# xmed-lab/GL-Fusion

Hardware: AMD Instinct MI355X
Metric: clips/sec fwd+bwd (B=4, 3 views x16x112x112) per GPU, weak scaling (higher is better)
Workload: dtype f32 (amax-scaled split-fp16 x3 MFMA, fp32 accumulate: fp32-equivalent); 1 GPU; C2: (B,V,T,H,W)=(4,3,16,112,112) per GPU, views 1/3/4, fp32 train() fwd + sum-BCE + bwd; global_batch_clips=4, frames_per_view_per_gpu=64, precision=f16x3, parallelism=single GPU, ranks_in_collective=1

## Files before the change

### gl-fusion_amd/csrc/norm.hip

```cpp
#include "stream_common.h"
#include "split_f16.h"

using namespace glf;

namespace {

constexpr int RT = 256;
constexpr int MAX_SLICES = 1024;

__host__ __device__ inline int n_slices_c(int rows, int c) {
    int s = (rows + 31) / 32;
    int cap = 524288 / (c > 0 ? c : 1);
    if (cap < 128) cap = 128;
    if (cap > MAX_SLICES) cap = MAX_SLICES;
    return s < 1 ? 1 : (s > cap ? cap : s);
}

struct Coef { const float* mean; const float* invstd; const float* gamma; const float* beta; };

struct OpStats {
    const float* x; int ldx;
    __device__ void operator()(int r, int c, float4& a, float4& b) const {
        a = *reinterpret_cast<const float4*>(x + (long long)r * ldx + c);
        b = make_float4(a.x * a.x, a.y * a.y, a.z * a.z, a.w * a.w);
    }
};
struct OpColsum {
    const float* dy; int ld;
    __device__ void operator()(int r, int c, float4& a, float4& b) const {
        a = *reinterpret_cast<const float4*>(dy + (long long)r * ld + c);
        b = make_float4(0.f, 0.f, 0.f, 0.f);
    }
};
__device__ __forceinline__ float bn_val(float x, float mu, float is, float ga, float be) { return (x - mu) * is * ga + be; }

struct OpBnBwd {
    const float* dy; int lddy; const float* x; int ldx; const float* y; int ldy;
    const float* mean; const float* invstd; const float* gamma; const float* beta; int relu;
    const unsigned char* mask; int c4;
    const float* dy2; int lddy2;
    __device__ void operator()(int r, int c, float4& a, float4& b) const {
        a = *reinterpret_cast<const float4*>(dy + (long long)r * lddy + c);
        if (dy2) {
            const float4 a2 = *reinterpret_cast<const float4*>(dy2 + (long long)r * lddy2 + c);
            a.x += a2.x; a.y += a2.y; a.z += a2.z; a.w += a2.w;
        }
        const float4 xx = *reinterpret_cast<const float4*>(x + (long long)r * ldx + c);
        const float4 mu = *reinterpret_cast<const float4*>(mean + c);
        const float4 is = *reinterpret_cast<const float4*>(invstd + c);
        if (relu && mask) {
            const unsigned m = mask[(long long)r * c4 + (c >> 2)];
            a.x = (m & 1u) ? a.x : 0.f; a.y = (m & 2u) ? a.y : 0.f; a.z = (m & 4u) ? a.z : 0.f; a.w = (m & 8u) ? a.w : 0.f;
        } else if (relu) {
            float4 yy;
            if (y) {
                yy = *reinterpret_cast<const float4*>(y + (long long)r * ldy + c);
            } else {
                const float4 ga = *reinterpret_cast<const float4*>(gamma + c);
                const float4 be = *reinterpret_cast<const float4*>(beta + c);
                yy = make_float4(bn_val(xx.x, mu.x, is.x, ga.x, be.x), bn_val(xx.y, mu.y, is.y, ga.y, be.y),
                                 bn_val(xx.z, mu.z, is.z, ga.z, be.z), bn_val(xx.w, mu.w, is.w, ga.w, be.w));
            }
            a.x = yy.x > 0.f ? a.x : 0.f; a.y = yy.y > 0.f ? a.y : 0.f;
            a.z = yy.z > 0.f ? a.z : 0.f; a.w = yy.w > 0.f ? a.w : 0.f;
        }
        b = make_float4(a.x * (xx.x - mu.x) * is.x, a.y * (xx.y - mu.y) * is.y,
                        a.z * (xx.z - mu.z) * is.z, a.w * (xx.w - mu.w) * is.w);
    }
};
struct OpLnParam {
    const float* dz; const float* w; const float* x; Coef bn; const float* row_mean; const float* row_rstd; int c_total;
    __device__ void operator()(int r, int c, float4& a, float4& b) const {
        const long long o = (long long)r * c_total + c;
        b = *reinterpret_cast<const float4*>(dz + o);
        const float4 ww = *reinterpret_cast<const float4*>(w + o);
        const float4 xx = *reinterpret_cast<const float4*>(x + o);
        const float4 mu = *reinterpret_cast<const float4*>(bn.mean + c);
        const float4 is = *reinterpret_cast<const float4*>(bn.invstd + c);
        const float4 ga = *reinterpret_cast<const float4*>(bn.gamma + c);
        const float4 be = *reinterpret_cast<const float4*>(bn.beta + c);
        const float m = row_mean[r], rs = row_rstd[r];
        const float u0 = (ww.x - mu.x) * is.x * ga.x + be.x + xx.x;
        const float u1 = (ww.y - mu.y) * is.y * ga.y + be.y + xx.y;
        const float u2 = (ww.z - mu.z) * is.z * ga.z + be.z + xx.z;
        const float u3 = (ww.w - mu.w) * is.w * ga.w + be.w + xx.w;
        a = make_float4(b.x * (u0 - m) * rs, b.y * (u1 - m) * rs, b.z * (u2 - m) * rs, b.w * (u3 - m) * rs);
    }
};

template <class Op>
__global__ __launch_bounds__(RT) void colreduce_kernel(Op op, int rows, int c, int slices, double* __restrict__ partial) {
    __shared__ double sh_a[RT * 4];
    __shared__ double sh_b[RT * 4];
    const int tid = threadIdx.x;
    const int c4 = c >> 2;
    const int tpr = c4 < RT ? c4 : RT;
    const int rpp = RT / tpr;
    const int ct = tid % tpr, rl = tid / tpr;
    const int slice = blockIdx.x;
    const int per = (rows + slices - 1) / slices;
    const int r0 = slice * per, r1 = min(rows, r0 + per);
    for (int cb = blockIdx.y * tpr; cb < c4; cb += gridDim.y * tpr) {
        const int cc = cb + ct;
        double a0 = 0, a1 = 0, a2 = 0, a3 = 0, b0 = 0, b1 = 0, b2 = 0, b3 = 0;
        if (cc < c4 && rl < rpp) {
            for (int r = r0 + rl; r < r1; r += rpp) {
                float4 a, b;
                op(r, cc * 4, a, b);
                a0 += a.x; a1 += a.y; a2 += a.z; a3 += a.w;
                b0 += b.x; b1 += b.y; b2 += b.z; b3 += b.w;
            }
        }
        sh_a[tid * 4 + 0] = a0; sh_a[tid * 4 + 1] = a1; sh_a[tid * 4 + 2] = a2; sh_a[tid * 4 + 3] = a3;
        sh_b[tid * 4 + 0] = b0; sh_b[tid * 4 + 1] = b1; sh_b[tid * 4 + 2] = b2; sh_b[tid * 4 + 3] = b3;
        __syncthreads();
        if (rl == 0 && cc < c4) {
            for (int q = 1; q < rpp; ++q) {
                const int o = (q * tpr + ct) * 4;
                a0 += sh_a[o]; a1 += sh_a[o + 1]; a2 += sh_a[o + 2]; a3 += sh_a[o + 3];
                b0 += sh_b[o]; b1 += sh_b[o + 1]; b2 += sh_b[o + 2]; b3 += sh_b[o + 3];
            }
            double* pa = partial + (long long)slice * c + cc * 4;
            double* pb = partial + (long long)(slices + slice) * c + cc * 4;
            pa[0] = a0; pa[1] = a1; pa[2] = a2; pa[3] = a3;
            pb[0] = b0; pb[1] = b1; pb[2] = b2; pb[3] = b3;
        }
        __syncthreads();
    }
}

__global__ __launch_bounds__(RT) void bnbwd_reduce_kernel(OpBnBwd op, int rows, int c, int slices, double* __restrict__ partial,
                                                          float* __restrict__ pmax) {
    __shared__ double sh_a[RT * 4];
    __shared__ double sh_b[RT * 4];
    __shared__ float sh_m[RT * 8];
    const int tid = threadIdx.x;
    const int c4 = c >> 2;
    const int tpr = c4 < RT ? c4 : RT;
    const int rpp = RT / tpr;
    const int ct = tid % tpr, rl = tid / tpr;
    const int slice = blockIdx.x;
    const int per = (rows + slices - 1) / slices;
    const int r0 = slice * per, r1 = min(rows, r0 + per);
    for (int cb = blockIdx.y * tpr; cb < c4; cb += gridDim.y * tpr) {
        const int cc = cb + ct;
        double a0 = 0, a1 = 0, a2 = 0, a3 = 0, b0 = 0, b1 = 0, b2 = 0, b3 = 0;
        float mg[4] = {0.f, 0.f, 0.f, 0.f}, mx[4] = {0.f, 0.f, 0.f, 0.f};
        if (cc < c4 && rl < rpp) {
            const float4 mu = *reinterpret_cast<const float4*>(op.mean + cc * 4);
            const float4 is = *reinterpret_cast<const float4*>(op.invstd + cc * 4);
            for (int r = r0 + rl; r < r1; r += rpp) {
                float4 a, b;
                op(r, cc * 4, a, b);
                a0 += a.x; a1 += a.y; a2 += a.z; a3 += a.w;
                b0 += b.x; b1 += b.y; b2 += b.z; b3 += b.w;
                const float4 xx = *reinterpret_cast<const float4*>(op.x + (long long)r * op.ldx + cc * 4);
                mg[0] = fmaxf(mg[0], fabsf(a.x)); mg[1] = fmaxf(mg[1], fabsf(a.y)); mg[2] = fmaxf(mg[2], fabsf(a.z)); mg[3] = fmaxf(mg[3], fabsf(a.w));
                mx[0] = fmaxf(mx[0], fabsf((xx.x - mu.x) * is.x)); mx[1] = fmaxf(mx[1], fabsf((xx.y - mu.y) * is.y));
                mx[2] = fmaxf(mx[2], fabsf((xx.z - mu.z) * is.z)); mx[3] = fmaxf(mx[3], fabsf((xx.w - mu.w) * is.w));
            }
        }
        sh_a[tid * 4 + 0] = a0; sh_a[tid * 4 + 1] = a1; sh_a[tid * 4 + 2] = a2; sh_a[tid * 4 + 3] = a3;
        sh_b[tid * 4 + 0] = b0; sh_b[tid * 4 + 1] = b1; sh_b[tid * 4 + 2] = b2; sh_b[tid * 4 + 3] = b3;
#pragma unroll
        for (int j = 0; j < 4; ++j) { sh_m[tid * 8 + j] = mg[j]; sh_m[tid * 8 + 4 + j] = mx[j]; }
        __syncthreads();
        if (rl == 0 && cc < c4) {
            for (int q = 1; q < rpp; ++q) {
                const int o = (q * tpr + ct) * 4;
                a0 += sh_a[o]; a1 += sh_a[o + 1]; a2 += sh_a[o + 2]; a3 += sh_a[o + 3];
                b0 += sh_b[o]; b1 += sh_b[o + 1]; b2 += sh_b[o + 2]; b3 += sh_b[o + 3];
#pragma unroll
                for (int j = 0; j < 4; ++j) { mg[j] = fmaxf(mg[j], sh_m[2 * o + j]); mx[j] = fmaxf(mx[j], sh_m[2 * o + 4 + j]); }
            }
            double* pa = partial + (long long)slice * c + cc * 4;
            double* pb = partial + (long long)(slices + slice) * c + cc * 4;
            pa[0] = a0; pa[1] = a1; pa[2] = a2; pa[3] = a3;
            pb[0] = b0; pb[1] = b1; pb[2] = b2; pb[3] = b3;
            *reinterpret_cast<float4*>(pmax + (long long)slice * c + cc * 4) = make_float4(mg[0], mg[1], mg[2], mg[3]);
            *reinterpret_cast<float4*>(pmax + (long long)(slices + slice) * c + cc * 4) = make_float4(mx[0], mx[1], mx[2], mx[3]);
        }
        __syncthreads();
    }
}

constexpr int FUSED_TPR = 16;
__host__ __device__ inline int fused_slices(int rows, int c) {
    const int c4 = c > 4 ? c / 4 : 1;
    const int tpr = c4 < FUSED_TPR ? c4 : FUSED_TPR;
    const int rpp = RT / tpr;
    int s = (rows + 16 * rpp - 1) / (16 * rpp);
    const int cblocks = (c4 + tpr - 1) / tpr;
    int cap = 1024 / cblocks;
    if (cap < 1) cap = 1;
    return s < 1 ? 1 : (s > cap ? cap : s);
}
template <bool HAS2, int RM>
__global__ __launch_bounds__(RT) void bnbwd_reduce_atomic_kernel(OpBnBwd op, int rows, int c, int slices, double* __restrict__ sums,
                                                                 float* __restrict__ cmax) {
    __shared__ float sh[RT * 8];
    const int tid = threadIdx.x;
    const int c4 = c >> 2;
    const int tpr = c4 < FUSED_TPR ? c4 : FUSED_TPR;
    const int rpp = RT / tpr;
    const int ct = tid % tpr, rl = tid / tpr;
    const int slice = blockIdx.x;
    const int per = (rows + slices - 1) / slices;
    const int r0 = slice * per, r1 = min(rows, r0 + per);
    for (int cb = blockIdx.y * tpr; cb < c4; cb += gridDim.y * tpr) {
        const int cc = cb + ct;
        float4 sa = make_float4(0.f, 0.f, 0.f, 0.f), sb = sa, mg = sa, mx = sa;
        if (cc < c4 && rl < rpp) {
            const int c0 = cc * 4;
            const float4 mu = *reinterpret_cast<const float4*>(op.mean + c0);
            const float4 is = *reinterpret_cast<const float4*>(op.invstd + c0);
            float4 ga = mu, be = mu;
            if (RM == 2) { ga = *reinterpret_cast<const float4*>(op.gamma + c0); be = *reinterpret_cast<const float4*>(op.beta + c0); }
            auto fold = [&](float4 a, const float4 a2, const float4 xx, const float4 yy, unsigned m) __attribute__((always_inline)) {
                if (HAS2) { a.x += a2.x; a.y += a2.y; a.z += a2.z; a.w += a2.w; }
                if (RM == 2) {
                    m = (bn_val(xx.x, mu.x, is.x, ga.x, be.x) > 0.f ? 1u : 0u) | (bn_val(xx.y, mu.y, is.y, ga.y, be.y) > 0.f ? 2u : 0u) |
                        (bn_val(xx.z, mu.z, is.z, ga.z, be.z) > 0.f ? 4u : 0u) | (bn_val(xx.w, mu.w, is.w, ga.w, be.w) > 0.f ? 8u : 0u);
                } else if (RM == 3) {
                    m = (yy.x > 0.f ? 1u : 0u) | (yy.y > 0.f ? 2u : 0u) | (yy.z > 0.f ? 4u : 0u) | (yy.w > 0.f ? 8u : 0u);
                }
                if (RM != 0) { a.x = (m & 1u) ? a.x : 0.f; a.y = (m & 2u) ? a.y : 0.f; a.z = (m & 4u) ? a.z : 0.f; a.w = (m & 8u) ? a.w : 0.f; }
                const float4 xh = make_float4((xx.x - mu.x) * is.x, (xx.y - mu.y) * is.y, (xx.z - mu.z) * is.z, (xx.w - mu.w) * is.w);
                sa.x += a.x; sa.y += a.y; sa.z += a.z; sa.w += a.w;
                sb.x += a.x * (xx.x - mu.x) * is.x; sb.y += a.y * (xx.y - mu.y) * is.y; sb.z += a.z * (xx.z - mu.z) * is.z; sb.w += a.w * (xx.w - mu.w) * is.w;
                if (cmax) {
                    mg.x = fmaxf(mg.x, fabsf(a.x)); mg.y = fmaxf(mg.y, fabsf(a.y)); mg.z = fmaxf(mg.z, fabsf(a.z)); mg.w = fmaxf(mg.w, fabsf(a.w));
                    mx.x = fmaxf(mx.x, fabsf(xh.x)); mx.y = fmaxf(mx.y, fabsf(xh.y)); mx.z = fmaxf(mx.z, fabsf(xh.z)); mx.w = fmaxf(mx.w, fabsf(xh.w));
                }
            };
            int r = r0 + rl;
            for (; r + 3 * rpp < r1; r += 4 * rpp) {
                float4 qa[4], qa2[4], qx[4], qy[4];
                unsigned m[4] = {15u, 15u, 15u, 15u};
#pragma unroll
                for (int u = 0; u < 4; ++u) {
                    const long long row = r + u * rpp;
                    qa[u] = *reinterpret_cast<const float4*>(op.dy + row * op.lddy + c0);
                    if (HAS2) qa2[u] = *reinterpret_cast<const float4*>(op.dy2 + row * op.lddy2 + c0);
                    qx[u] = *reinterpret_cast<const float4*>(op.x + row * op.ldx + c0);
                    if (RM == 3) qy[u] = *reinterpret_cast<const float4*>(op.y + row * op.ldy + c0);
                    if (RM == 1) m[u] = op.mask[row * op.c4 + cc];
                }
                __builtin_amdgcn_sched_barrier(0);
#pragma unroll
                for (int u = 0; u < 4; ++u) fold(qa[u], HAS2 ? qa2[u] : qa[u], qx[u], RM == 3 ? qy[u] : qx[u], m[u]);
            }
            for (; r < r1; r += rpp) {
                const long long row = r;
                const float4 qa = *reinterpret_cast<const float4*>(op.dy + row * op.lddy + c0);
                const float4 qa2 = HAS2 ? *reinterpret_cast<const float4*>(op.dy2 + row * op.lddy2 + c0) : qa;
                const float4 qx = *reinterpret_cast<const float4*>(op.x + row * op.ldx + c0);
                const float4 qy = RM == 3 ? *reinterpret_cast<const float4*>(op.y + row * op.ldy + c0) : qx;
                const unsigned m = RM == 1 ? op.mask[row * op.c4 + cc] : 15u;
                fold(qa, qa2, qx, qy, m);
            }
        }
        const int ncol = tpr * 4;
        for (int pass = 0; pass < (cmax ? 2 : 1); ++pass) {
            if (rl < rpp) {
                const float4 u = pass == 0 ? sa : mg, v = pass == 0 ? sb : mx;
                float* d0 = sh + (0 * rpp + rl) * ncol + ct * 4;
                float* d1 = sh + (1 * rpp + rl) * ncol + ct * 4;
                d0[0] = u.x; d0[1] = u.y; d0[2] = u.z; d0[3] = u.w;
                d1[0] = v.x; d1[1] = v.y; d1[2] = v.z; d1[3] = v.w;
            }
            __syncthreads();
            for (int idx = tid; idx < 2 * ncol; idx += RT) {
                const int st = idx / ncol, col = idx - st * ncol;
                const int gc = cb * 4 + col;
                if (gc < c) {
                    if (pass == 0) {
                        double d = 0;
                        for (int q = 0; q < rpp; ++q) d += sh[(st * rpp + q) * ncol + col];
                        atomicAdd(sums + st * c + gc, d);
                    } else {
                        float m = 0.f;
                        for (int q = 0; q < rpp; ++q) m = fmaxf(m, sh[(st * rpp + q) * ncol + col]);
                        if (m > 0.f) atomicMax(reinterpret_cast<unsigned*>(cmax + st * c + gc), __float_as_uint(m));
                    }
                }
            }
            __syncthreads();
        }
    }
}

constexpr int FIN_CH = 16, FIN_LANES = 16;

__device__ __forceinline__ void fold_partials(const double* __restrict__ partial, int slices, int c, int ch, int lane,
                                              double& s, double& q, double* sh) {
    s = 0; q = 0;
    if (ch < c) {
        double s1 = 0, q1 = 0, s2 = 0, q2 = 0, s3 = 0, q3 = 0;
        int i = lane;
        for (; i + 3 * FIN_LANES < slices; i += 4 * FIN_LANES) {
            s += partial[(long long)i * c + ch];                     q += partial[(long long)(slices + i) * c + ch];
            s1 += partial[(long long)(i + FIN_LANES) * c + ch];      q1 += partial[(long long)(slices + i + FIN_LANES) * c + ch];
            s2 += partial[(long long)(i + 2 * FIN_LANES) * c + ch];  q2 += partial[(long long)(slices + i + 2 * FIN_LANES) * c + ch];
            s3 += partial[(long long)(i + 3 * FIN_LANES) * c + ch];  q3 += partial[(long long)(slices + i + 3 * FIN_LANES) * c + ch];
        }
        for (; i < slices; i += FIN_LANES) {
            s += partial[(long long)i * c + ch];
            q += partial[(long long)(slices + i) * c + ch];
        }
        s += (s1 + s2) + s3; q += (q1 + q2) + q3;
    }
    const int t = threadIdx.x;
    sh[t] = s; sh[256 + t] = q;
    __syncthreads();
    if (lane == 0) {
        for (int l = 1; l < FIN_LANES; ++l) { s += sh[t + l * FIN_CH]; q += sh[256 + t + l * FIN_CH]; }
    }
}

__global__ __launch_bounds__(256) void bn_stats_finalize(const double* __restrict__ partial, int slices, int c, int rows, float eps,
                                                         float momentum, float* mean, float* invstd, float* rmean, float* rvar, long long* nbt) {
    __shared__ double sh[512];
    const int cx = threadIdx.x % FIN_CH, lane = threadIdx.x / FIN_CH;
    const int ch = blockIdx.x * FIN_CH + cx;
    double s, q;
    fold_partials(partial, slices, c, ch, lane, s, q, sh);
    if (lane != 0 || ch >= c) return;
    if (ch == 0 && nbt) *nbt += 1;
    const double m = s / rows;
    double var = q / rows - m * m;
    if (var < 0) var = 0;
    mean[ch] = (float)m;
    invstd[ch] = (float)(1.0 / sqrt(var + (double)eps));
    if (rmean) {
        const double unb = rows > 1 ? var * rows / (rows - 1) : var;
        rmean[ch] = (1.f - momentum) * rmean[ch] + momentum * (float)m;
        rvar[ch] = (1.f - momentum) * rvar[ch] + momentum * (float)unb;
    }
}

__global__ __launch_bounds__(256) void sum_finalize(const double* __restrict__ partial, int slices, int c, float* out_a, float* out_b) {
    __shared__ double sh[512];
    const int cx = threadIdx.x % FIN_CH, lane = threadIdx.x / FIN_CH;
    const int ch = blockIdx.x * FIN_CH + cx;
    double s, q;
    fold_partials(partial, slices, c, ch, lane, s, q, sh);
    if (lane != 0 || ch >= c) return;
    if (out_a) out_a[ch] = (float)s;
    if (out_b) out_b[ch] = (float)q;
}

__global__ __launch_bounds__(256) void bnbwd_finalize(const double* __restrict__ partial, const float* __restrict__ pmax, int slices, int c,
                                                      const float* __restrict__ gamma, const float* __restrict__ invstd, float inv_n,
                                                      int training, float* out_a, float* out_b, float* __restrict__ bound,
                                                      float* __restrict__ keep) {
    __shared__ double sh[512];
    __shared__ float shm[512];
    const int cx = threadIdx.x % FIN_CH, lane = threadIdx.x / FIN_CH;
    const int ch = blockIdx.x * FIN_CH + cx;
    double s, q;
    fold_partials(partial, slices, c, ch, lane, s, q, sh);
    float mg = 0.f, mx = 0.f;
    if (ch < c) {
        float g1 = 0.f, x1 = 0.f, g2 = 0.f, x2 = 0.f, g3 = 0.f, x3 = 0.f;
        int i = lane;
        for (; i + 3 * FIN_LANES < slices; i += 4 * FIN_LANES) {
            mg = fmaxf(mg, pmax[(long long)i * c + ch]);                      mx = fmaxf(mx, pmax[(long long)(slices + i) * c + ch]);
            g1 = fmaxf(g1, pmax[(long long)(i + FIN_LANES) * c + ch]);        x1 = fmaxf(x1, pmax[(long long)(slices + i + FIN_LANES) * c + ch]);
            g2 = fmaxf(g2, pmax[(long long)(i + 2 * FIN_LANES) * c + ch]);    x2 = fmaxf(x2, pmax[(long long)(slices + i + 2 * FIN_LANES) * c + ch]);
            g3 = fmaxf(g3, pmax[(long long)(i + 3 * FIN_LANES) * c + ch]);    x3 = fmaxf(x3, pmax[(long long)(slices + i + 3 * FIN_LANES) * c + ch]);
        }
        for (; i < slices; i += FIN_LANES) {
            mg = fmaxf(mg, pmax[(long long)i * c + ch]);
            mx = fmaxf(mx, pmax[(long long)(slices + i) * c + ch]);
        }
        mg = fmaxf(fmaxf(mg, g1), fmaxf(g2, g3)); mx = fmaxf(fmaxf(mx, x1), fmaxf(x2, x3));
    }
    shm[threadIdx.x] = mg; shm[256 + threadIdx.x] = mx;
    __syncthreads();
    if (lane != 0 || ch >= c) return;
    for (int l = 1; l < FIN_LANES; ++l) { mg = fmaxf(mg, shm[threadIdx.x + l * FIN_CH]); mx = fmaxf(mx, shm[256 + threadIdx.x + l * FIN_CH]); }
    if (out_a) out_a[ch] = (float)s;
    if (out_b) out_b[ch] = (float)q;
    if (keep) { keep[ch] = (float)s; keep[c + ch] = (float)q; }
    const float k = fabsf(gamma[ch] * invstd[ch]);
    const float b = 1.0001f * k * (training ? mg + inv_n * (fabsf((float)s) + mx * fabsf((float)q)) : mg);
    if (b > 0.f && b < 3.0e38f) atomicMax(reinterpret_cast<unsigned*>(bound), __float_as_uint(b));
}

__global__ void bn_replay_kernel(const float* __restrict__ mean, const float* __restrict__ invstd, int rows, float eps, float momentum,
                                 float* rmean, float* rvar, long long* nbt, int c) {
    const int ch = blockIdx.x * blockDim.x + threadIdx.x;
    if (ch == 0 && nbt) *nbt += 1;
    if (ch >= c) return;
    const double is = (double)invstd[ch];
    double var = 1.0 / (is * is) - (double)eps;
    if (var < 0) var = 0;
    const double unb = rows > 1 ? var * rows / (rows - 1) : var;
    rmean[ch] = (1.f - momentum) * rmean[ch] + momentum * mean[ch];
    rvar[ch] = (1.f - momentum) * rvar[ch] + momentum * (float)unb;
}

__global__ void bn_eval_coeffs_kernel(const float* rm, const float* rv, float eps, float* mean, float* invstd, int c) {
    const int ch = blockIdx.x * blockDim.x + threadIdx.x;
    if (ch >= c) return;
    mean[ch] = rm[ch];
    invstd[ch] = 1.0f / sqrtf(rv[ch] + eps);
}


__global__ __launch_bounds__(256) void bn_apply_kernel(const float* __restrict__ x, int ldx, const float* __restrict__ res, int ldr,
                                                       float* __restrict__ y, int ldy, Coef k, long long total4, int c4, int relu,
                                                       float* __restrict__ amax_out, unsigned char* __restrict__ mask) {
    float am = 0.f;
    for (long long i = blockIdx.x * (long long)blockDim.x + threadIdx.x; i < total4; i += (long long)gridDim.x * blockDim.x) {
        const long long r = i / c4;
        const int c = (int)(i - r * c4) * 4;
        const float4 xx = *reinterpret_cast<const float4*>(x + r * ldx + c);
        const float4 mu = *reinterpret_cast<const float4*>(k.mean + c);
        const float4 is = *reinterpret_cast<const float4*>(k.invstd + c);
        const float4 ga = *reinterpret_cast<const float4*>(k.gamma + c);
        const float4 be = *reinterpret_cast<const float4*>(k.beta + c);
        float4 o = make_float4(bn_val(xx.x, mu.x, is.x, ga.x, be.x), bn_val(xx.y, mu.y, is.y, ga.y, be.y),
                               bn_val(xx.z, mu.z, is.z, ga.z, be.z), bn_val(xx.w, mu.w, is.w, ga.w, be.w));
        if (res) {
            const float4 rr = *reinterpret_cast<const float4*>(res + r * ldr + c);
            o.x += rr.x; o.y += rr.y; o.z += rr.z; o.w += rr.w;
        }
        if (mask) mask[i] = (unsigned char)((o.x > 0.f) | ((o.y > 0.f) << 1) | ((o.z > 0.f) << 2) | ((o.w > 0.f) << 3));
        if (relu) { o.x = fmaxf(o.x, 0.f); o.y = fmaxf(o.y, 0.f); o.z = fmaxf(o.z, 0.f); o.w = fmaxf(o.w, 0.f); }
        *reinterpret_cast<float4*>(y + r * ldy + c) = o;
        am = fmaxf(fmaxf(am, fmaxf(fabsf(o.x), fabsf(o.y))), fmaxf(fabsf(o.z), fabsf(o.w)));
    }
    if (amax_out) block_amax(am, amax_out);
}

constexpr int APPLY_MAX_C = 4096;
__global__ __launch_bounds__(256) void bn_apply_sums_kernel(const float* __restrict__ x, int ldx, const float* __restrict__ res, int ldr,
                                                            float* __restrict__ y, int ldy, const double* __restrict__ sums, int rows, int c,
                                                            float eps, float momentum, const float* __restrict__ gamma, const float* __restrict__ beta,
                                                            float* __restrict__ mean_out, float* __restrict__ invstd_out, float* rmean, float* rvar,
                                                            long long* nbt, long long total4, int c4, int relu, float* __restrict__ amax_out,
                                                            unsigned char* __restrict__ mask, const float* __restrict__ colmax) {
    extern __shared__ __attribute__((aligned(16))) float s_coef[];
    __shared__ float s_bound[4];
    float* s_mean = s_coef;
    float* s_is = s_coef + c;
    float bound = 0.f;
    for (int ch = threadIdx.x; ch < c; ch += blockDim.x) {
        const double m = sums[ch] / rows;
        double var = sums[c + ch] / rows - m * m;
        if (var < 0) var = 0;
        const float mf = (float)m, isf = (float)(1.0 / sqrt(var + (double)eps));
        s_mean[ch] = mf; s_is[ch] = isf;
        if (colmax) bound = fmaxf(bound, fabsf(gamma[ch]) * isf * (colmax[ch] + fabsf(mf)) + fabsf(beta[ch]));
        if (blockIdx.x == 0) {
            mean_out[ch] = mf; invstd_out[ch] = isf;
            if (rmean) {
                const double unb = rows > 1 ? var * rows / (rows - 1) : var;
                rmean[ch] = (1.f - momentum) * rmean[ch] + momentum * (float)m;
                rvar[ch] = (1.f - momentum) * rvar[ch] + momentum * (float)unb;
            }
        }
    }
    if (blockIdx.x == 0 && threadIdx.x == 0 && nbt) *nbt += 1;
    float sc = 1.f, sc_inv = 1.f;
    if (colmax) {
#pragma unroll
        for (int o = 32; o > 0; o >>= 1) bound = fmaxf(bound, __shfl_xor(bound, o, 64));
        if ((threadIdx.x & 63) == 0) s_bound[threadIdx.x >> 6] = bound;
    }
    __syncthreads();
    if (colmax) {
        bound = 1.0001f * fmaxf(fmaxf(s_bound[0], s_bound[1]), fmaxf(s_bound[2], s_bound[3]));
        if (blockIdx.x == 0 && threadIdx.x == 0) *amax_out = bound;
        pow2_scale(&bound, sc, sc_inv);
    }
    float am = 0.f;
    for (long long i = blockIdx.x * (long long)blockDim.x + threadIdx.x; i < total4; i += (long long)gridDim.x * blockDim.x) {
        const long long r = i / c4;
        const int cc = (int)(i - r * c4) * 4;
        const float4 xx = *reinterpret_cast<const float4*>(x + r * ldx + cc);
        const float4 mu = *reinterpret_cast<const float4*>(s_mean + cc);
        const float4 is = *reinterpret_cast<const float4*>(s_is + cc);
        const float4 ga = *reinterpret_cast<const float4*>(gamma + cc);
        const float4 be = *reinterpret_cast<const float4*>(beta + cc);
        float4 o = make_float4(bn_val(xx.x, mu.x, is.x, ga.x, be.x), bn_val(xx.y, mu.y, is.y, ga.y, be.y),
                               bn_val(xx.z, mu.z, is.z, ga.z, be.z), bn_val(xx.w, mu.w, is.w, ga.w, be.w));
        if (res) {
            const float4 rr = *reinterpret_cast<const float4*>(res + r * ldr + cc);
            o.x += rr.x; o.y += rr.y; o.z += rr.z; o.w += rr.w;
        }
        if (mask) mask[i] = (unsigned char)((o.x > 0.f) | ((o.y > 0.f) << 1) | ((o.z > 0.f) << 2) | ((o.w > 0.f) << 3));
        if (relu) { o.x = fmaxf(o.x, 0.f); o.y = fmaxf(o.y, 0.f); o.z = fmaxf(o.z, 0.f); o.w = fmaxf(o.w, 0.f); }
        if (colmax) {
            const SplitH sp = split4h(o, sc);
            const float2 h = __builtin_bit_cast(float2, sp.h), l = __builtin_bit_cast(float2, sp.l);
            o = make_float4(h.x, h.y, l.x, l.y);
        } else {
            am = fmaxf(fmaxf(am, fmaxf(fabsf(o.x), fabsf(o.y))), fmaxf(fabsf(o.z), fabsf(o.w)));
        }
        *reinterpret_cast<float4*>(y + r * ldy + cc) = o;
    }
    if (amax_out && !colmax) block_amax(am, amax_out);
}

__global__ __launch_bounds__(256) void bn_bwd_apply_kernel(const float* __restrict__ dy, int lddy, const float* __restrict__ x, int ldx,
                                                           const float* __restrict__ y, int ldy, Coef k,
                                                           const float* __restrict__ sum_dy, const float* __restrict__ sum_dyx,
                                                           float* __restrict__ dx, int lddx, float* __restrict__ dres, int lddres,
                                                           long long total4, int c4, int relu, int training, float inv_n,
                                                           float* __restrict__ amax_out, int packed, const unsigned char* __restrict__ mask,
                                                           const float* __restrict__ dy2, int lddy2, const double* __restrict__ fsums,
                                                           const float* __restrict__ fmax, float* __restrict__ out_dbeta, float* __restrict__ out_dgamma,
                                                           int c) {
    extern __shared__ __attribute__((aligned(16))) float s_fin[];
    __shared__ float s_bound[4];
    float bound_local = 0.f;
    if (fsums) {
        for (int ch = threadIdx.x; ch < c; ch += blockDim.x) {
            const float a = (float)fsums[ch], b = (float)fsums[c + ch];
            s_fin[ch] = a; s_fin[c + ch] = b;
            if (blockIdx.x == 0) { if (out_dbeta) out_dbeta[ch] = a; if (out_dgamma) out_dgamma[ch] = b; }
            if (packed) {
                const float kk = fabsf(k.gamma[ch] * k.invstd[ch]);
                const float bb = 1.0001f * kk * (training ? fmax[ch] + inv_n * (fabsf(a) + fmax[c + ch] * fabsf(b)) : fmax[ch]);
                if (bb < 3.0e38f) bound_local = fmaxf(bound_local, bb);
            }
        }
        if (packed) {
#pragma unroll
            for (int o = 32; o > 0; o >>= 1) bound_local = fmaxf(bound_local, __shfl_xor(bound_local, o, 64));
            if ((threadIdx.x & 63) == 0) s_bound[threadIdx.x >> 6] = bound_local;
        }
        __syncthreads();
        sum_dy = s_fin; sum_dyx = s_fin + c;
    }
    float am = 0.f, sc = 1.f, sc_inv = 1.f;
    if (packed && fsums) {
        float bnd = fmaxf(fmaxf(s_bound[0], s_bound[1]), fmaxf(s_bound[2], s_bound[3]));
        if (blockIdx.x == 0 && threadIdx.x == 0) *amax_out = bnd;
        pow2_scale(&bnd, sc, sc_inv);
    } else if (packed) pow2_scale(amax_out, sc, sc_inv);
    for (long long i = blockIdx.x * (long long)blockDim.x + threadIdx.x; i < total4; i += (long long)gridDim.x * blockDim.x) {
        const long long r = i / c4;
        const int c = (int)(i - r * c4) * 4;
        float4 g = *reinterpret_cast<const float4*>(dy + r * lddy + c);
        if (dy2) {
            const float4 g2 = *reinterpret_cast<const float4*>(dy2 + r * lddy2 + c);
            g.x += g2.x; g.y += g2.y; g.z += g2.z; g.w += g2.w;
        }
        const float4 is = *reinterpret_cast<const float4*>(k.invstd + c);
        const float4 ga = *reinterpret_cast<const float4*>(k.gamma + c);
        float4 xx = make_float4(0.f, 0.f, 0.f, 0.f), mu = xx;
        if (training || (relu && !y && !mask)) {
            xx = *reinterpret_cast<const float4*>(x + r * ldx + c);
            mu = *reinterpret_cast<const float4*>(k.mean + c);
        }
        if (relu && mask) {
            const unsigned m = mask[i];
            g.x = (m & 1u) ? g.x : 0.f; g.y = (m & 2u) ? g.y : 0.f; g.z = (m & 4u) ? g.z : 0.f; g.w = (m & 8u) ? g.w : 0.f;
        } else if (relu) {
            float4 yy;
            if (y) {
                yy = *reinterpret_cast<const float4*>(y + r * ldy + c);
            } else {
                const float4 be = *reinterpret_cast<const float4*>(k.beta + c);
                yy = make_float4(bn_val(xx.x, mu.x, is.x, ga.x, be.x), bn_val(xx.y, mu.y, is.y, ga.y, be.y),
                                 bn_val(xx.z, mu.z, is.z, ga.z, be.z), bn_val(xx.w, mu.w, is.w, ga.w, be.w));
            }
            g.x = yy.x > 0.f ? g.x : 0.f; g.y = yy.y > 0.f ? g.y : 0.f;
            g.z = yy.z > 0.f ? g.z : 0.f; g.w = yy.w > 0.f ? g.w : 0.f;
        }
        if (dres) *reinterpret_cast<float4*>(dres + r * lddres + c) = g;
        float4 o;
        if (training) {
            const float4 s1 = *reinterpret_cast<const float4*>(sum_dy + c);
            const float4 s2 = *reinterpret_cast<const float4*>(sum_dyx + c);
            o.x = ga.x * is.x * (g.x - inv_n * (s1.x + (xx.x - mu.x) * is.x * s2.x));
            o.y = ga.y * is.y * (g.y - inv_n * (s1.y + (xx.y - mu.y) * is.y * s2.y));
            o.z = ga.z * is.z * (g.z - inv_n * (s1.z + (xx.z - mu.z) * is.z * s2.z));
            o.w = ga.w * is.w * (g.w - inv_n * (s1.w + (xx.w - mu.w) * is.w * s2.w));
        } else {
            o = make_float4(g.x * ga.x * is.x, g.y * ga.y * is.y, g.z * ga.z * is.z, g.w * ga.w * is.w);
        }
        if (packed) {
            const SplitH sp = split4h(o, sc);
            const float2 h = __builtin_bit_cast(float2, sp.h), l = __builtin_bit_cast(float2, sp.l);
            o = make_float4(h.x, h.y, l.x, l.y);
        } else {
            am = fmaxf(fmaxf(am, fmaxf(fabsf(o.x), fabsf(o.y))), fmaxf(fabsf(o.z), fabsf(o.w)));
        }
        *reinterpret_cast<float4*>(dx + r * lddx + c) = o;
    }
    if (amax_out && !packed) block_amax(am, amax_out);
}

constexpr int LN_NV = 8;

template <bool BWD>
__global__ __launch_bounds__(256) void bn_res_ln_kernel(const float* __restrict__ w, const float* __restrict__ x, Coef bn,
                                                        const float* __restrict__ ln_g, const float* __restrict__ ln_b, float eps,
                                                        float* __restrict__ z, float* __restrict__ row_mean, float* __restrict__ row_rstd,
                                                        const float* __restrict__ dz, float* __restrict__ du, int rows, int c,
                                                        float* __restrict__ amax_out) {
    const int lane = threadIdx.x & 63;
    const int row = blockIdx.x * 4 + (threadIdx.x >> 6);
    if (row >= rows) return;
    const int c4 = c >> 2;
    const long long base = (long long)row * c;
    float4 u[LN_NV];
    float s = 0.f;
#pragma unroll
    for (int v = 0; v < LN_NV; ++v) {
        const int cc = lane + 64 * v;
        if (cc < c4) {
            const int ch = cc * 4;
            const float4 ww = *reinterpret_cast<const float4*>(w + base + ch);
            const float4 xx = *reinterpret_cast<const float4*>(x + base + ch);
            const float4 mu = *reinterpret_cast<const float4*>(bn.mean + ch);
            const float4 is = *reinterpret_cast<const float4*>(bn.invstd + ch);
            const float4 ga = *reinterpret_cast<const float4*>(bn.gamma + ch);
            const float4 be = *reinterpret_cast<const float4*>(bn.beta + ch);
            u[v] = make_float4((ww.x - mu.x) * is.x * ga.x + be.x + xx.x, (ww.y - mu.y) * is.y * ga.y + be.y + xx.y,
                               (ww.z - mu.z) * is.z * ga.z + be.z + xx.z, (ww.w - mu.w) * is.w * ga.w + be.w + xx.w);
            s += (u[v].x + u[v].y) + (u[v].z + u[v].w);
        } else {
            u[v] = make_float4(0.f, 0.f, 0.f, 0.f);
        }
    }
    float mean, rstd;
    if (!BWD) {
        mean = wave_sum(s) / c;
        float q = 0.f;
#pragma unroll
        for (int v = 0; v < LN_NV; ++v)
            if (lane + 64 * v < c4) {
                const float a = u[v].x - mean, b = u[v].y - mean, cc2 = u[v].z - mean, d = u[v].w - mean;
                q += (a * a + b * b) + (cc2 * cc2 + d * d);
            }
        rstd = 1.0f / sqrtf(wave_sum(q) / c + eps);
        if (lane == 0) { row_mean[row] = mean; row_rstd[row] = rstd; }
        float am = 0.f;
#pragma unroll
        for (int v = 0; v < LN_NV; ++v) {
            const int cc = lane + 64 * v;
            if (cc < c4) {
                const int ch = cc * 4;
                const float4 g = *reinterpret_cast<const float4*>(ln_g + ch);
                const float4 b = *reinterpret_cast<const float4*>(ln_b + ch);
                const float4 o = make_float4((u[v].x - mean) * rstd * g.x + b.x, (u[v].y - mean) * rstd * g.y + b.y,
                                             (u[v].z - mean) * rstd * g.z + b.z, (u[v].w - mean) * rstd * g.w + b.w);
                *reinterpret_cast<float4*>(z + base + ch) = o;
                am = fmaxf(fmaxf(am, fmaxf(fabsf(o.x), fabsf(o.y))), fmaxf(fabsf(o.z), fabsf(o.w)));
            }
        }
        if (amax_out) {
#pragma unroll
            for (int o = 32; o > 0; o >>= 1) am = fmaxf(am, __shfl_xor(am, o, 64));
            if (lane == 0 && am > *reinterpret_cast<volatile float*>(amax_out)) atomicMax(reinterpret_cast<unsigned*>(amax_out), __float_as_uint(am));
        }
    } else {
        mean = row_mean[row]; rstd = row_rstd[row];
        float4 gz[LN_NV];
        float s1 = 0.f, s2 = 0.f;
#pragma unroll
        for (int v = 0; v < LN_NV; ++v) {
            const int cc = lane + 64 * v;
            if (cc < c4) {
                const int ch = cc * 4;
                const float4 d = *reinterpret_cast<const float4*>(dz + base + ch);
                const float4 g = *reinterpret_cast<const float4*>(ln_g + ch);
                gz[v] = make_float4(d.x * g.x, d.y * g.y, d.z * g.z, d.w * g.w);
                u[v] = make_float4((u[v].x - mean) * rstd, (u[v].y - mean) * rstd, (u[v].z - mean) * rstd, (u[v].w - mean) * rstd);
                s1 += (gz[v].x + gz[v].y) + (gz[v].z + gz[v].w);
                s2 += (gz[v].x * u[v].x + gz[v].y * u[v].y) + (gz[v].z * u[v].z + gz[v].w * u[v].w);
            } else {
                gz[v] = make_float4(0.f, 0.f, 0.f, 0.f);
            }
        }
        const float m1 = wave_sum(s1) / c, m2 = wave_sum(s2) / c;
#pragma unroll
        for (int v = 0; v < LN_NV; ++v) {
            const int cc = lane + 64 * v;
            if (cc < c4)
                *reinterpret_cast<float4*>(du + base + cc * 4) =
                    make_float4(rstd * (gz[v].x - m1 - u[v].x * m2), rstd * (gz[v].y - m1 - u[v].y * m2),
                                rstd * (gz[v].z - m1 - u[v].z * m2), rstd * (gz[v].w - m1 - u[v].w * m2));
        }
    }
}

template <class Op>
int launch_colreduce(Op op, int rows, int c, double* ws, hipStream_t s) {
    const int slices = n_slices_c(rows, c);
    const int c4 = c / 4, tpr = c4 < RT ? c4 : RT;
    hipLaunchKernelGGL((colreduce_kernel<Op>), dim3(slices, (c4 + tpr - 1) / tpr), dim3(RT), 0, s, op, rows, c, slices, ws);
    return glf::check_launch("colreduce");
}

}

extern "C" size_t glf_bn_workspace(int rows, int c) {
    return (size_t)3 * MAX_SLICES * (size_t)(c > 0 ? c : 0) + (size_t)2 * (c > 0 ? c : 0);
}

#define REQ_C4(c) GLF_REQUIRE((c) > 0 && ((c) % 4) == 0, GLF_ERR_BAD_SHAPE, "channel count must be a positive multiple of 4 (got %d)", (c))
#define REQ_LD(ld, name) GLF_REQUIRE(((ld) % 4) == 0, GLF_ERR_BAD_SHAPE, name " must be a multiple of 4")

extern "C" int glf_bn_stats(const float* x, int ldx, int rows, int c, float eps, float momentum,
                            float* mean, float* invstd, float* running_mean, float* running_var,
                            int64_t* num_batches_tracked, double* workspace, glf_stream_t s) {
    if (int rc = glf::ensure_init()) return rc;
    GLF_REQUIRE(x && mean && invstd && workspace, GLF_ERR_NULL, "bn_stats: null argument");
    GLF_REQUIRE(rows > 0, GLF_ERR_BAD_SHAPE, "bn_stats: rows must be > 0");
    REQ_C4(c); REQ_AL(x, "x"); REQ_LD(ldx, "ldx");
    GLF_REQUIRE((running_mean == nullptr) == (running_var == nullptr), GLF_ERR_NULL, "bn_stats: running_mean/var must both be set or both NULL");
    if (int rc = launch_colreduce(OpStats{x, ldx}, rows, c, workspace, glf::S(s))) return rc;
    hipLaunchKernelGGL(bn_stats_finalize, dim3((c + FIN_CH - 1) / FIN_CH), dim3(256), 0, glf::S(s), workspace, n_slices_c(rows, c), c, rows,
                       eps, momentum, mean, invstd, running_mean, running_var, reinterpret_cast<long long*>(num_batches_tracked));
    return glf::check_launch("bn_stats_finalize");
}

extern "C" int glf_bn_stats_from_sums(const double* sums, int rows, int c, float eps, float momentum, float* mean, float* invstd,
                                      float* running_mean, float* running_var, int64_t* num_batches_tracked, glf_stream_t s) {
    if (int rc = glf::ensure_init()) return rc;
    GLF_REQUIRE(sums && mean && invstd, GLF_ERR_NULL, "bn_stats_from_sums: null argument");
    GLF_REQUIRE(rows > 0 && c > 0, GLF_ERR_BAD_SHAPE, "bn_stats_from_sums: rows and c must be > 0");
    GLF_REQUIRE((running_mean == nullptr) == (running_var == nullptr), GLF_ERR_NULL, "bn_stats_from_sums: running_mean/var must both be set or both NULL");
    hipLaunchKernelGGL(bn_stats_finalize, dim3((c + FIN_CH - 1) / FIN_CH), dim3(256), 0, glf::S(s), sums, 1, c, rows,
                       eps, momentum, mean, invstd, running_mean, running_var, reinterpret_cast<long long*>(num_batches_tracked));
    return glf::check_launch("bn_stats_from_sums");
}

extern "C" int glf_bn_replay_running(const float* mean, const float* invstd, int rows, int c, float eps, float momentum,
                                     float* running_mean, float* running_var, int64_t* num_batches_tracked, glf_stream_t s) {
    if (int rc = glf::ensure_init()) return rc;
    GLF_REQUIRE(mean && invstd && running_mean && running_var, GLF_ERR_NULL, "bn_replay_running: null argument");
    GLF_REQUIRE(rows > 0 && c > 0, GLF_ERR_BAD_SHAPE, "bn_replay_running: rows and c must be > 0");
    hipLaunchKernelGGL(bn_replay_kernel, dim3((c + 255) / 256), dim3(256), 0, glf::S(s), mean, invstd, rows, eps, momentum,
                       running_mean, running_var, reinterpret_cast<long long*>(num_batches_tracked), c);
    return glf::check_launch("bn_replay_running");
}

extern "C" int glf_bn_eval_coeffs(const float* rm, const float* rv, float eps, float* mean, float* invstd, int c, glf_stream_t s) {
    GLF_REQUIRE(rm && rv && mean && invstd, GLF_ERR_NULL, "bn_eval_coeffs: null argument");
    GLF_REQUIRE(c > 0, GLF_ERR_BAD_SHAPE, "bn_eval_coeffs: c must be > 0");
    hipLaunchKernelGGL(bn_eval_coeffs_kernel, dim3((c + 255) / 256), dim3(256), 0, glf::S(s), rm, rv, eps, mean, invstd, c);
    return glf::check_launch("bn_eval_coeffs");
}

extern "C" int glf_bn_apply(const float* x, int ldx, const float* residual, int ldr, float* y, int ldy,
                            const float* mean, const float* invstd, const float* gamma, const float* beta,
                            int rows, int c, int relu, float* amax_out, uint8_t* relu_mask, glf_stream_t s) {
    if (int rc = glf::ensure_init()) return rc;
    GLF_REQUIRE(x && y && mean && invstd && gamma && beta, GLF_ERR_NULL, "bn_apply: null argument");
    GLF_REQUIRE(rows > 0, GLF_ERR_BAD_SHAPE, "bn_apply: rows must be > 0");
    REQ_C4(c); REQ_AL(x, "x"); REQ_AL(y, "y"); REQ_LD(ldx, "ldx"); REQ_LD(ldy, "ldy");
    if (residual) { REQ_AL(residual, "residual"); REQ_LD(ldr, "ldr"); }
    const long long total4 = (long long)rows * (c / 4);
    hipLaunchKernelGGL(bn_apply_kernel, dim3(stream_grid(total4, 256)), dim3(256), 0, glf::S(s), x, ldx, residual, ldr, y, ldy,
                       Coef{mean, invstd, gamma, beta}, total4, c / 4, relu, amax_out, relu_mask);
    return glf::check_launch("bn_apply");
}

extern "C" int glf_bn_apply_from_sums(const float* x, int ldx, const float* residual, int ldr, float* y, int ldy, const double* sums,
                                      int rows, int c, float eps, float momentum, const float* gamma, const float* beta,
                                      float* mean, float* invstd, float* running_mean, float* running_var, int64_t* num_batches_tracked,
                                      int relu, float* amax_out, uint8_t* relu_mask, const float* colmax, glf_stream_t s) {
    if (int rc = glf::ensure_init()) return rc;
    GLF_REQUIRE(x && y && sums && mean && invstd && gamma && beta, GLF_ERR_NULL, "bn_apply_from_sums: null argument");
    GLF_REQUIRE(!colmax || (amax_out && !residual && y != x), GLF_ERR_BAD_SHAPE, "bn_apply_from_sums: the packed output (colmax) needs amax_out, no residual and y != x");
    GLF_REQUIRE(rows > 0, GLF_ERR_BAD_SHAPE, "bn_apply_from_sums: rows must be > 0");
    REQ_C4(c); REQ_AL(x, "x"); REQ_AL(y, "y"); REQ_LD(ldx, "ldx"); REQ_LD(ldy, "ldy");
    GLF_REQUIRE(c <= APPLY_MAX_C, GLF_ERR_UNSUPPORTED, "bn_apply_from_sums: C must be <= %d (use glf_bn_stats_from_sums + glf_bn_apply)", APPLY_MAX_C);
    GLF_REQUIRE((running_mean == nullptr) == (running_var == nullptr), GLF_ERR_NULL, "bn_apply_from_sums: running_mean/var must both be set or both NULL");
    if (residual) { REQ_AL(residual, "residual"); REQ_LD(ldr, "ldr"); }
    const long long total4 = (long long)rows * (c / 4);
    hipLaunchKernelGGL(bn_apply_sums_kernel, dim3(stream_grid(total4, 256)), dim3(256), (size_t)2 * c * sizeof(float), glf::S(s), x, ldx, residual, ldr, y, ldy, sums, rows, c,
                       eps, momentum, gamma, beta, mean, invstd, running_mean, running_var, reinterpret_cast<long long*>(num_batches_tracked),
                       total4, c / 4, relu, amax_out, relu_mask, colmax);
    return glf::check_launch("bn_apply_from_sums");
}

extern "C" int glf_bn_bwd(const float* dy, int lddy, const float* x, int ldx, const float* y, int ldy,
                          const float* mean, const float* invstd, const float* gamma, const float* beta,
                          float* dx, int lddx, float* dres, int lddres, float* dgamma, float* dbeta,
                          int rows, int c, int relu, int training, double* workspace, float* amax_out, int packed_dx,
                          const uint8_t* relu_mask, const float* dy2, int lddy2, double* fused_sums, glf_stream_t s) {
    if (int rc = glf::ensure_init()) return rc;
    GLF_REQUIRE(dy && x && mean && invstd && gamma && dx && (workspace || fused_sums), GLF_ERR_NULL, "bn_bwd: null argument");
    if (relu_mask) y = nullptr;
    GLF_REQUIRE(!packed_dx || amax_out, GLF_ERR_NULL, "bn_bwd: packed_dx needs amax_out (a zeroed device float that receives the bound the image is scaled with)");
    GLF_REQUIRE(!relu || y || beta || relu_mask, GLF_ERR_NULL, "bn_bwd: relu != 0 needs relu_mask, y (the forward output) or beta (to recompute its sign from x)");
    GLF_REQUIRE(rows > 0, GLF_ERR_BAD_SHAPE, "bn_bwd: rows must be > 0");
    REQ_C4(c); REQ_AL(dy, "dy"); REQ_AL(x, "x"); REQ_AL(dx, "dx"); REQ_LD(lddy, "lddy"); REQ_LD(ldx, "ldx"); REQ_LD(lddx, "lddx");
    if (relu && y) { REQ_AL(y, "y"); REQ_LD(ldy, "ldy"); }
    if (dres) { REQ_AL(dres, "dres"); REQ_LD(lddres, "lddres"); }
    if (dy2) { REQ_AL(dy2, "dy2"); REQ_LD(lddy2, "lddy2"); }
    const OpBnBwd op{dy, lddy, x, ldx, y, ldy, mean, invstd, gamma, beta, relu, relu_mask, c / 4, dy2, lddy2};
    const long long total4f = (long long)rows * (c / 4);
    const int phase = packed_dx >= 2 ? packed_dx : 0;
    GLF_REQUIRE(packed_dx >= 0 && packed_dx <= 3, GLF_ERR_BAD_SHAPE, "bn_bwd: packed_dx must be 0 .. 3");
    GLF_REQUIRE(!phase || (workspace && fused_sums), GLF_ERR_NULL, "bn_bwd: packed_dx = 2 / 3 needs the workspace and fused_sums (2 c floats kept from half 2 to half 3)");
    GLF_REQUIRE(phase != 2 || (dgamma && dbeta), GLF_ERR_NULL, "bn_bwd: packed_dx = 2 needs dgamma and dbeta");
    float* keep = phase ? reinterpret_cast<float*>(fused_sums) : (float*)nullptr;
    if (!phase && fused_sums && c <= APPLY_MAX_C) {
        float* fmax = reinterpret_cast<float*>(fused_sums + (size_t)2 * c);
        const int fs = fused_slices(rows, c);
        const int c4 = c / 4, tpr = c4 < FUSED_TPR ? c4 : FUSED_TPR;
        const dim3 rgrid(fs, (c4 + tpr - 1) / tpr);
        float* rmax = packed_dx ? fmax : (float*)nullptr;
        const int rm = !op.relu ? 0 : (op.mask ? 1 : (op.y ? 3 : 2));
#define GLF_BNR(H2, RM_) hipLaunchKernelGGL((bnbwd_reduce_atomic_kernel<H2, RM_>), rgrid, dim3(RT), 0, glf::S(s), op, rows, c, fs, fused_sums, rmax)
        if (op.dy2) { if (rm == 0) GLF_BNR(true, 0); else if (rm == 1) GLF_BNR(true, 1); else if (rm == 2) GLF_BNR(true, 2); else GLF_BNR(true, 3); }
        else { if (rm == 0) GLF_BNR(false, 0); else if (rm == 1) GLF_BNR(false, 1); else if (rm == 2) GLF_BNR(false, 2); else GLF_BNR(false, 3); }
#undef GLF_BNR
        if (int rc = glf::check_launch("bn_bwd_reduce(fused)")) return rc;
        hipLaunchKernelGGL(bn_bwd_apply_kernel, dim3(stream_grid(total4f, 256)), dim3(256), (size_t)2 * c * sizeof(float), glf::S(s), dy, lddy, x, ldx, y, ldy,
                           Coef{mean, invstd, gamma, beta}, (const float*)nullptr, (const float*)nullptr, dx, lddx, dres, lddres, total4f, c / 4, relu, training,
                           1.0f / (float)rows, amax_out, packed_dx, relu_mask, dy2, lddy2, fused_sums, fmax, dbeta, dgamma, c);
        return glf::check_launch("bn_bwd_apply(fused)");
    }
    GLF_REQUIRE(workspace, GLF_ERR_NULL, "bn_bwd: the three-launch form needs the workspace");
    const int slices = n_slices_c(rows, c);
    float* sums = reinterpret_cast<float*>(workspace + (size_t)2 * slices * c);
    float* s_dy = dbeta ? dbeta : sums;
    float* s_dyx = dgamma ? dgamma : sums + c;
    if (phase == 3) {
        s_dy = keep; s_dyx = keep + c;
    } else if (packed_dx) {
        float* pmax = reinterpret_cast<float*>(workspace + (size_t)2 * slices * c + (size_t)2 * c);
        const int c4 = c / 4, tpr = c4 < RT ? c4 : RT;
        hipLaunchKernelGGL(bnbwd_reduce_kernel, dim3(slices, (c4 + tpr - 1) / tpr), dim3(RT), 0, glf::S(s), op, rows, c, slices, workspace, pmax);
        if (int rc = glf::check_launch("bn_bwd_reduce")) return rc;
        hipLaunchKernelGGL(bnbwd_finalize, dim3((c + FIN_CH - 1) / FIN_CH), dim3(256), 0, glf::S(s), workspace, pmax, slices, c, gamma, invstd,
                           1.0f / (float)rows, training, s_dy, s_dyx, amax_out, keep);
    } else {
        if (int rc = launch_colreduce(op, rows, c, workspace, glf::S(s))) return rc;
        hipLaunchKernelGGL(sum_finalize, dim3((c + FIN_CH - 1) / FIN_CH), dim3(256), 0, glf::S(s), workspace, slices, c, s_dy, s_dyx);
    }
    if (int rc = glf::check_launch("bn_bwd_finalize")) return rc;
    if (phase == 2) return GLF_OK;
    const long long total4 = (long long)rows * (c / 4);
    hipLaunchKernelGGL(bn_bwd_apply_kernel, dim3(stream_grid(total4, 256)), dim3(256), 0, glf::S(s), dy, lddy, x, ldx, y, ldy,
                       Coef{mean, invstd, gamma, beta}, s_dy, s_dyx, dx, lddx, dres, lddres, total4, c / 4, relu, training,
                       1.0f / (float)rows, amax_out, packed_dx, relu_mask, dy2, lddy2, (const double*)nullptr, (const float*)nullptr, (float*)nullptr,
                       (float*)nullptr, c);
    return glf::check_launch("bn_bwd_apply");
}

extern "C" int glf_colsum(const float* dy, int lddy, float* db, int rows, int c, double* workspace, glf_stream_t s) {
    if (int rc = glf::ensure_init()) return rc;
    GLF_REQUIRE(dy && db && workspace, GLF_ERR_NULL, "colsum: null argument");
    GLF_REQUIRE(rows > 0, GLF_ERR_BAD_SHAPE, "colsum: rows must be > 0");
    REQ_C4(c); REQ_AL(dy, "dy"); REQ_LD(lddy, "lddy");
    if (int rc = launch_colreduce(OpColsum{dy, lddy}, rows, c, workspace, glf::S(s))) return rc;
    hipLaunchKernelGGL(sum_finalize, dim3((c + FIN_CH - 1) / FIN_CH), dim3(256), 0, glf::S(s), workspace, n_slices_c(rows, c), c, db, (float*)nullptr);
    return glf::check_launch("colsum_finalize");
}

extern "C" int glf_bn_res_ln_fwd(const float* w, const float* x, const float* bn_mean, const float* bn_invstd,
                                 const float* bn_gamma, const float* bn_beta, const float* ln_gamma,
                                 const float* ln_beta, float ln_eps, float* z, float* row_mean, float* row_rstd,
                                 int rows, int c, float* amax_out, glf_stream_t s) {
    if (int rc = glf::ensure_init()) return rc;
    GLF_REQUIRE(w && x && bn_mean && bn_invstd && bn_gamma && bn_beta && ln_gamma && ln_beta && z && row_mean && row_rstd,
                GLF_ERR_NULL, "bn_res_ln_fwd: null argument");
    GLF_REQUIRE(rows > 0, GLF_ERR_BAD_SHAPE, "bn_res_ln_fwd: rows must be > 0");
    REQ_C4(c); GLF_REQUIRE(c <= 64 * 4 * LN_NV, GLF_ERR_UNSUPPORTED, "bn_res_ln: C must be <= %d", 64 * 4 * LN_NV);
    REQ_AL(w, "w"); REQ_AL(x, "x"); REQ_AL(z, "z");
    hipLaunchKernelGGL((bn_res_ln_kernel<false>), dim3((rows + 3) / 4), dim3(256), 0, glf::S(s), w, x,
                       Coef{bn_mean, bn_invstd, bn_gamma, bn_beta}, ln_gamma, ln_beta, ln_eps, z, row_mean, row_rstd,
                       (const float*)nullptr, (float*)nullptr, rows, c, amax_out);
    return glf::check_launch("bn_res_ln_fwd");
}

extern "C" int glf_bn_res_ln_bwd(const float* dz, const float* w, const float* x, const float* bn_mean,
                                 const float* bn_invstd, const float* bn_gamma, const float* bn_beta,
                                 const float* ln_gamma, const float* row_mean, const float* row_rstd,
                                 float* du, float* dln_gamma, float* dln_beta, int rows, int c,
                                 double* workspace, glf_stream_t s) {
    if (int rc = glf::ensure_init()) return rc;
    GLF_REQUIRE(dz && w && x && bn_mean && bn_invstd && bn_gamma && bn_beta && ln_gamma && row_mean && row_rstd && du &&
                dln_gamma && dln_beta && workspace, GLF_ERR_NULL, "bn_res_ln_bwd: null argument");
    GLF_REQUIRE(rows > 0, GLF_ERR_BAD_SHAPE, "bn_res_ln_bwd: rows must be > 0");
    REQ_C4(c); GLF_REQUIRE(c <= 64 * 4 * LN_NV, GLF_ERR_UNSUPPORTED, "bn_res_ln: C must be <= %d", 64 * 4 * LN_NV);
    REQ_AL(dz, "dz"); REQ_AL(w, "w"); REQ_AL(x, "x"); REQ_AL(du, "du");
    const Coef bn{bn_mean, bn_invstd, bn_gamma, bn_beta};
    hipLaunchKernelGGL((bn_res_ln_kernel<true>), dim3((rows + 3) / 4), dim3(256), 0, glf::S(s), w, x, bn, ln_gamma,
                       (const float*)nullptr, 0.f, (float*)nullptr, const_cast<float*>(row_mean), const_cast<float*>(row_rstd),
                       dz, du, rows, c, (float*)nullptr);
    if (int rc = glf::check_launch("bn_res_ln_bwd")) return rc;
    if (int rc = launch_colreduce(OpLnParam{dz, w, x, bn, row_mean, row_rstd, c}, rows, c, workspace, glf::S(s))) return rc;
    hipLaunchKernelGGL(sum_finalize, dim3((c + FIN_CH - 1) / FIN_CH), dim3(256), 0, glf::S(s), workspace, n_slices_c(rows, c), c, dln_gamma, dln_beta);
    return glf::check_launch("ln_param_finalize");
}
```

Before: 17.29 clips/s.

## Restructure BN apply kernels into column-tiled row-strided form and write dres in reduce

Replaces the flat grid-stride BN forward and backward apply kernels with a column-tiled layout. Each thread owns a fixed column group and walks rows in unrolled batches of four, so the per-channel coefficients are loaded once and the per-element div/mod indexing goes away. The fused backward reduce kernel now writes the masked, summed gradient (dres) during its pass. The apply step can then read that single tensor instead of re-reading dy, dy2 and the mask. It adds template variants and a new launch helper, and shifts more stores into the reduce pass.

```diff
diff --git a/gl-fusion_amd/csrc/norm.hip b/gl-fusion_amd/csrc/norm.hip
--- a/gl-fusion_amd/csrc/norm.hip
+++ b/gl-fusion_amd/csrc/norm.hip
@@ -195,9 +195,9 @@
     if (cap < 1) cap = 1;
     return s < 1 ? 1 : (s > cap ? cap : s);
 }
-template <bool HAS2, int RM>
+template <bool HAS2, int RM, bool WRES>
 __global__ __launch_bounds__(RT) void bnbwd_reduce_atomic_kernel(OpBnBwd op, int rows, int c, int slices, double* __restrict__ sums,
-                                                                 float* __restrict__ cmax) {
+                                                                 float* __restrict__ cmax, float* __restrict__ dres, int lddres) {
     __shared__ float sh[RT * 8];
     const int tid = threadIdx.x;
     const int c4 = c >> 2;
@@ -216,7 +216,7 @@
             const float4 is = *reinterpret_cast<const float4*>(op.invstd + c0);
             float4 ga = mu, be = mu;
             if (RM == 2) { ga = *reinterpret_cast<const float4*>(op.gamma + c0); be = *reinterpret_cast<const float4*>(op.beta + c0); }
-            auto fold = [&](float4 a, const float4 a2, const float4 xx, const float4 yy, unsigned m) __attribute__((always_inline)) {
+            auto fold = [&](long long row, float4 a, const float4 a2, const float4 xx, const float4 yy, unsigned m) __attribute__((always_inline)) {
                 if (HAS2) { a.x += a2.x; a.y += a2.y; a.z += a2.z; a.w += a2.w; }
                 if (RM == 2) {
                     m = (bn_val(xx.x, mu.x, is.x, ga.x, be.x) > 0.f ? 1u : 0u) | (bn_val(xx.y, mu.y, is.y, ga.y, be.y) > 0.f ? 2u : 0u) |
@@ -225,6 +225,7 @@
                     m = (yy.x > 0.f ? 1u : 0u) | (yy.y > 0.f ? 2u : 0u) | (yy.z > 0.f ? 4u : 0u) | (yy.w > 0.f ? 8u : 0u);
                 }
                 if (RM != 0) { a.x = (m & 1u) ? a.x : 0.f; a.y = (m & 2u) ? a.y : 0.f; a.z = (m & 4u) ? a.z : 0.f; a.w = (m & 8u) ? a.w : 0.f; }
+                if (WRES) *reinterpret_cast<float4*>(dres + row * lddres + c0) = a;
                 const float4 xh = make_float4((xx.x - mu.x) * is.x, (xx.y - mu.y) * is.y, (xx.z - mu.z) * is.z, (xx.w - mu.w) * is.w);
                 sa.x += a.x; sa.y += a.y; sa.z += a.z; sa.w += a.w;
                 sb.x += a.x * (xx.x - mu.x) * is.x; sb.y += a.y * (xx.y - mu.y) * is.y; sb.z += a.z * (xx.z - mu.z) * is.z; sb.w += a.w * (xx.w - mu.w) * is.w;
@@ -248,7 +249,7 @@
                 }
                 __builtin_amdgcn_sched_barrier(0);
 #pragma unroll
-                for (int u = 0; u < 4; ++u) fold(qa[u], HAS2 ? qa2[u] : qa[u], qx[u], RM == 3 ? qy[u] : qx[u], m[u]);
+                for (int u = 0; u < 4; ++u) fold(r + u * rpp, qa[u], HAS2 ? qa2[u] : qa[u], qx[u], RM == 3 ? qy[u] : qx[u], m[u]);
             }
             for (; r < r1; r += rpp) {
                 const long long row = r;
@@ -257,7 +258,7 @@
                 const float4 qx = *reinterpret_cast<const float4*>(op.x + row * op.ldx + c0);
                 const float4 qy = RM == 3 ? *reinterpret_cast<const float4*>(op.y + row * op.ldy + c0) : qx;
                 const unsigned m = RM == 1 ? op.mask[row * op.c4 + cc] : 15u;
-                fold(qa, qa2, qx, qy, m);
+                fold(row, qa, qa2, qx, qy, m);
             }
         }
         const int ncol = tpr * 4;
@@ -408,182 +409,50 @@
     invstd[ch] = 1.0f / sqrtf(rv[ch] + eps);
 }
 
-
-__global__ __launch_bounds__(256) void bn_apply_kernel(const float* __restrict__ x, int ldx, const float* __restrict__ res, int ldr,
-                                                       float* __restrict__ y, int ldy, Coef k, long long total4, int c4, int relu,
-                                                       float* __restrict__ amax_out, unsigned char* __restrict__ mask) {
+constexpr int APPLY_TPR = 16, APPLY_TPR_WIDE = 64;
+constexpr int APPLY_MAXCOL = APPLY_TPR_WIDE * 4;
+
+struct ColGrid { int tpr, cblocks, slices; };
+inline ColGrid col_grid(int rows, int c) {
+    const int c4 = c / 4;
+    const int tpr = c4 >= APPLY_TPR_WIDE ? APPLY_TPR_WIDE : (c4 < APPLY_TPR ? c4 : APPLY_TPR);
+    const int rpp = 256 / tpr;
+    const int cblocks = (c4 + tpr - 1) / tpr;
+    long long s = stream_grid((long long)rows * c4, 256) / cblocks;
+    const int smax = (rows + rpp - 1) / rpp;
+    if (s > smax) s = smax;
+    if (s < 1) s = 1;
+    return {tpr, cblocks, (int)s};
+}
+inline dim3 col_dim(const ColGrid& g) { return dim3((unsigned)g.slices * (unsigned)g.cblocks); }
+
+struct ColLane { int cb, slice, cc, c0, r, r1, rpp; bool live; };
+__device__ __forceinline__ ColLane col_lane(int rows, int c4, int tpr, int cblocks, int slices) {
+    ColLane L;
+    L.rpp = 256 / tpr;
+    const int ct = threadIdx.x % tpr, rl = threadIdx.x / tpr;
+    L.cb = blockIdx.x % cblocks; L.slice = blockIdx.x / cblocks;
+    const int per = (rows + slices - 1) / slices;
+    const int r0 = L.slice * per;
+    L.r1 = min(rows, r0 + per);
+    L.r = r0 + rl;
+    L.cc = L.cb * tpr + ct; L.c0 = L.cc * 4;
+    L.live = L.cc < c4 && rl < L.rpp;
+    return L;
+}
+
+template <bool RES>
+__device__ __forceinline__ float bn_apply_rows(const ColLane& L, const float* __restrict__ x, int ldx, const float* __restrict__ res, int ldr,
+                                               float* __restrict__ y, int ldy, const float4 mu, const float4 is, const float4 ga, const float4 be,
+                                               int c4, int relu, unsigned char* __restrict__ mask, bool packed, float sc) {
     float am = 0.f;
-    for (long long i = blockIdx.x * (long long)blockDim.x + threadIdx.x; i < total4; i += (long long)gridDim.x * blockDim.x) {
-        const long long r = i / c4;
-        const int c = (int)(i - r * c4) * 4;
-        const float4 xx = *reinterpret_cast<const float4*>(x + r * ldx + c);
-        const float4 mu = *reinterpret_cast<const float4*>(k.mean + c);
-        const float4 is = *reinterpret_cast<const float4*>(k.invstd + c);
-        const float4 ga = *reinterpret_cast<const float4*>(k.gamma + c);
-        const float4 be = *reinterpret_cast<const float4*>(k.beta + c);
+    const int c0 = L.c0, cc = L.cc, rpp = L.rpp;
+    auto emit = [&](long long row, const float4 xx, const float4 rr) __attribute__((always_inline)) {
         float4 o = make_float4(bn_val(xx.x, mu.x, is.x, ga.x, be.x), bn_val(xx.y, mu.y, is.y, ga.y, be.y),
                                bn_val(xx.z, mu.z, is.z, ga.z, be.z), bn_val(xx.w, mu.w, is.w, ga.w, be.w));
-        if (res) {
-            const float4 rr = *reinterpret_cast<const float4*>(res + r * ldr + c);
-            o.x += rr.x; o.y += rr.y; o.z += rr.z; o.w += rr.w;
-        }
-        if (mask) mask[i] = (unsigned char)((o.x > 0.f) | ((o.y > 0.f) << 1) | ((o.z > 0.f) << 2) | ((o.w > 0.f) << 3));
+        if (RES) { o.x += rr.x; o.y += rr.y; o.z += rr.z; o.w += rr.w; }
+        if (mask) mask[row * c4 + cc] = (unsigned char)((o.x > 0.f) | ((o.y > 0.f) << 1) | ((o.z > 0.f) << 2) | ((o.w > 0.f) << 3));
         if (relu) { o.x = fmaxf(o.x, 0.f); o.y = fmaxf(o.y, 0.f); o.z = fmaxf(o.z, 0.f); o.w = fmaxf(o.w, 0.f); }
-        *reinterpret_cast<float4*>(y + r * ldy + c) = o;
-        am = fmaxf(fmaxf(am, fmaxf(fabsf(o.x), fabsf(o.y))), fmaxf(fabsf(o.z), fabsf(o.w)));
-    }
-    if (amax_out) block_amax(am, amax_out);
-}
-
-constexpr int APPLY_MAX_C = 4096;
-__global__ __launch_bounds__(256) void bn_apply_sums_kernel(const float* __restrict__ x, int ldx, const float* __restrict__ res, int ldr,
-                                                            float* __restrict__ y, int ldy, const double* __restrict__ sums, int rows, int c,
-                                                            float eps, float momentum, const float* __restrict__ gamma, const float* __restrict__ beta,
-                                                            float* __restrict__ mean_out, float* __restrict__ invstd_out, float* rmean, float* rvar,
-                                                            long long* nbt, long long total4, int c4, int relu, float* __restrict__ amax_out,
-                                                            unsigned char* __restrict__ mask, const float* __restrict__ colmax) {
-    extern __shared__ __attribute__((aligned(16))) float s_coef[];
-    __shared__ float s_bound[4];
-    float* s_mean = s_coef;
-    float* s_is = s_coef + c;
-    float bound = 0.f;
-    for (int ch = threadIdx.x; ch < c; ch += blockDim.x) {
-        const double m = sums[ch] / rows;
-        double var = sums[c + ch] / rows - m * m;
-        if (var < 0) var = 0;
-        const float mf = (float)m, isf = (float)(1.0 / sqrt(var + (double)eps));
-        s_mean[ch] = mf; s_is[ch] = isf;
-        if (colmax) bound = fmaxf(bound, fabsf(gamma[ch]) * isf * (colmax[ch] + fabsf(mf)) + fabsf(beta[ch]));
-        if (blockIdx.x == 0) {
-            mean_out[ch] = mf; invstd_out[ch] = isf;
-            if (rmean) {
-                const double unb = rows > 1 ? var * rows / (rows - 1) : var;
-                rmean[ch] = (1.f - momentum) * rmean[ch] + momentum * (float)m;
-                rvar[ch] = (1.f - momentum) * rvar[ch] + momentum * (float)unb;
-            }
-        }
-    }
-    if (blockIdx.x == 0 && threadIdx.x == 0 && nbt) *nbt += 1;
-    float sc = 1.f, sc_inv = 1.f;
-    if (colmax) {
-#pragma unroll
-        for (int o = 32; o > 0; o >>= 1) bound = fmaxf(bound, __shfl_xor(bound, o, 64));
-        if ((threadIdx.x & 63) == 0) s_bound[threadIdx.x >> 6] = bound;
-    }
-    __syncthreads();
-    if (colmax) {
-        bound = 1.0001f * fmaxf(fmaxf(s_bound[0], s_bound[1]), fmaxf(s_bound[2], s_bound[3]));
-        if (blockIdx.x == 0 && threadIdx.x == 0) *amax_out = bound;
-        pow2_scale(&bound, sc, sc_inv);
-    }
-    float am = 0.f;
-    for (long long i = blockIdx.x * (long long)blockDim.x + threadIdx.x; i < total4; i += (long long)gridDim.x * blockDim.x) {
-        const long long r = i / c4;
-        const int cc = (int)(i - r * c4) * 4;
-        const float4 xx = *reinterpret_cast<const float4*>(x + r * ldx + cc);
-        const float4 mu = *reinterpret_cast<const float4*>(s_mean + cc);
-        const float4 is = *reinterpret_cast<const float4*>(s_is + cc);
-        const float4 ga = *reinterpret_cast<const float4*>(gamma + cc);
-        const float4 be = *reinterpret_cast<const float4*>(beta + cc);
-        float4 o = make_float4(bn_val(xx.x, mu.x, is.x, ga.x, be.x), bn_val(xx.y, mu.y, is.y, ga.y, be.y),
-                               bn_val(xx.z, mu.z, is.z, ga.z, be.z), bn_val(xx.w, mu.w, is.w, ga.w, be.w));
-        if (res) {
-            const float4 rr = *reinterpret_cast<const float4*>(res + r * ldr + cc);
-            o.x += rr.x; o.y += rr.y; o.z += rr.z; o.w += rr.w;
-        }
-        if (mask) mask[i] = (unsigned char)((o.x > 0.f) | ((o.y > 0.f) << 1) | ((o.z > 0.f) << 2) | ((o.w > 0.f) << 3));
-        if (relu) { o.x = fmaxf(o.x, 0.f); o.y = fmaxf(o.y, 0.f); o.z = fmaxf(o.z, 0.f); o.w = fmaxf(o.w, 0.f); }
-        if (colmax) {
-            const SplitH sp = split4h(o, sc);
-            const float2 h = __builtin_bit_cast(float2, sp.h), l = __builtin_bit_cast(float2, sp.l);
-            o = make_float4(h.x, h.y, l.x, l.y);
-        } else {
-            am = fmaxf(fmaxf(am, fmaxf(fabsf(o.x), fabsf(o.y))), fmaxf(fabsf(o.z), fabsf(o.w)));
-        }
-        *reinterpret_cast<float4*>(y + r * ldy + cc) = o;
-    }
-    if (amax_out && !colmax) block_amax(am, amax_out);
-}
-
-__global__ __launch_bounds__(256) void bn_bwd_apply_kernel(const float* __restrict__ dy, int lddy, const float* __restrict__ x, int ldx,
-                                                           const float* __restrict__ y, int ldy, Coef k,
-                                                           const float* __restrict__ sum_dy, const float* __restrict__ sum_dyx,
-                                                           float* __restrict__ dx, int lddx, float* __restrict__ dres, int lddres,
-                                                           long long total4, int c4, int relu, int training, float inv_n,
-                                                           float* __restrict__ amax_out, int packed, const unsigned char* __restrict__ mask,
-                                                           const float* __restrict__ dy2, int lddy2, const double* __restrict__ fsums,
-                                                           const float* __restrict__ fmax, float* __restrict__ out_dbeta, float* __restrict__ out_dgamma,
-                                                           int c) {
-    extern __shared__ __attribute__((aligned(16))) float s_fin[];
-    __shared__ float s_bound[4];
-    float bound_local = 0.f;
-    if (fsums) {
-        for (int ch = threadIdx.x; ch < c; ch += blockDim.x) {
-            const float a = (float)fsums[ch], b = (float)fsums[c + ch];
-            s_fin[ch] = a; s_fin[c + ch] = b;
-            if (blockIdx.x == 0) { if (out_dbeta) out_dbeta[ch] = a; if (out_dgamma) out_dgamma[ch] = b; }
-            if (packed) {
-                const float kk = fabsf(k.gamma[ch] * k.invstd[ch]);
-                const float bb = 1.0001f * kk * (training ? fmax[ch] + inv_n * (fabsf(a) + fmax[c + ch] * fabsf(b)) : fmax[ch]);
-                if (bb < 3.0e38f) bound_local = fmaxf(bound_local, bb);
-            }
-        }
-        if (packed) {
-#pragma unroll
-            for (int o = 32; o > 0; o >>= 1) bound_local = fmaxf(bound_local, __shfl_xor(bound_local, o, 64));
-            if ((threadIdx.x & 63) == 0) s_bound[threadIdx.x >> 6] = bound_local;
-        }
-        __syncthreads();
-        sum_dy = s_fin; sum_dyx = s_fin + c;
-    }
-    float am = 0.f, sc = 1.f, sc_inv = 1.f;
-    if (packed && fsums) {
-        float bnd = fmaxf(fmaxf(s_bound[0], s_bound[1]), fmaxf(s_bound[2], s_bound[3]));
-        if (blockIdx.x == 0 && threadIdx.x == 0) *amax_out = bnd;
-        pow2_scale(&bnd, sc, sc_inv);
-    } else if (packed) pow2_scale(amax_out, sc, sc_inv);
-    for (long long i = blockIdx.x * (long long)blockDim.x + threadIdx.x; i < total4; i += (long long)gridDim.x * blockDim.x) {
-        const long long r = i / c4;
-        const int c = (int)(i - r * c4) * 4;
-        float4 g = *reinterpret_cast<const float4*>(dy + r * lddy + c);
-        if (dy2) {
-            const float4 g2 = *reinterpret_cast<const float4*>(dy2 + r * lddy2 + c);
-            g.x += g2.x; g.y += g2.y; g.z += g2.z; g.w += g2.w;
-        }
-        const float4 is = *reinterpret_cast<const float4*>(k.invstd + c);
-        const float4 ga = *reinterpret_cast<const float4*>(k.gamma + c);
-        float4 xx = make_float4(0.f, 0.f, 0.f, 0.f), mu = xx;
-        if (training || (relu && !y && !mask)) {
-            xx = *reinterpret_cast<const float4*>(x + r * ldx + c);
-            mu = *reinterpret_cast<const float4*>(k.mean + c);
-        }
-        if (relu && mask) {
-            const unsigned m = mask[i];
-            g.x = (m & 1u) ? g.x : 0.f; g.y = (m & 2u) ? g.y : 0.f; g.z = (m & 4u) ? g.z : 0.f; g.w = (m & 8u) ? g.w : 0.f;
-        } else if (relu) {
-            float4 yy;
-            if (y) {
-                yy = *reinterpret_cast<const float4*>(y + r * ldy + c);
-            } else {
-                const float4 be = *reinterpret_cast<const float4*>(k.beta + c);
-                yy = make_float4(bn_val(xx.x, mu.x, is.x, ga.x, be.x), bn_val(xx.y, mu.y, is.y, ga.y, be.y),
-                                 bn_val(xx.z, mu.z, is.z, ga.z, be.z), bn_val(xx.w, mu.w, is.w, ga.w, be.w));
-            }
-            g.x = yy.x > 0.f ? g.x : 0.f; g.y = yy.y > 0.f ? g.y : 0.f;
-            g.z = yy.z > 0.f ? g.z : 0.f; g.w = yy.w > 0.f ? g.w : 0.f;
-        }
-        if (dres) *reinterpret_cast<float4*>(dres + r * lddres + c) = g;
-        float4 o;
-        if (training) {
-            const float4 s1 = *reinterpret_cast<const float4*>(sum_dy + c);
-            const float4 s2 = *reinterpret_cast<const float4*>(sum_dyx + c);
-            o.x = ga.x * is.x * (g.x - inv_n * (s1.x + (xx.x - mu.x) * is.x * s2.x));
-            o.y = ga.y * is.y * (g.y - inv_n * (s1.y + (xx.y - mu.y) * is.y * s2.y));
-            o.z = ga.z * is.z * (g.z - inv_n * (s1.z + (xx.z - mu.z) * is.z * s2.z));
-            o.w = ga.w * is.w * (g.w - inv_n * (s1.w + (xx.w - mu.w) * is.w * s2.w));
-        } else {
-            o = make_float4(g.x * ga.x * is.x, g.y * ga.y * is.y, g.z * ga.z * is.z, g.w * ga.w * is.w);
-        }
         if (packed) {
             const SplitH sp = split4h(o, sc);
             const float2 h = __builtin_bit_cast(float2, sp.h), l = __builtin_bit_cast(float2, sp.l);
@@ -591,9 +460,228 @@
         } else {
             am = fmaxf(fmaxf(am, fmaxf(fabsf(o.x), fabsf(o.y))), fmaxf(fabsf(o.z), fabsf(o.w)));
         }
-        *reinterpret_cast<float4*>(dx + r * lddx + c) = o;
-    }
-    if (amax_out && !packed) block_amax(am, amax_out);
+        *reinterpret_cast<float4*>(y + row * ldy + c0) = o;
+    };
+    int r = L.r;
+    for (; r + 3 * rpp < L.r1; r += 4 * rpp) {
+        float4 qx[4], qr[4];
+#pragma unroll
+        for (int u = 0; u < 4; ++u) {
+            const long long row = r + u * rpp;
+            qx[u] = *reinterpret_cast<const float4*>(x + row * ldx + c0);
+            if (RES) qr[u] = *reinterpret_cast<const float4*>(res + row * ldr + c0);
+        }
+        __builtin_amdgcn_sched_barrier(0);
+#pragma unroll
+        for (int u = 0; u < 4; ++u) emit(r + u * rpp, qx[u], RES ? qr[u] : qx[u]);
+    }
+    for (; r < L.r1; r += rpp) {
+        const long long row = r;
+        const float4 qx = *reinterpret_cast<const float4*>(x + row * ldx + c0);
+        const float4 qr = RES ? *reinterpret_cast<const float4*>(res + row * ldr + c0) : qx;
+        emit(row, qx, qr);
+    }
+    return am;
+}
+
+template <bool RES>
+__global__ __launch_bounds__(256) void bn_apply_kernel(const float* __restrict__ x, int ldx, const float* __restrict__ res, int ldr,
+                                                       float* __restrict__ y, int ldy, Coef k, int rows, int c4, int tpr, int cblocks,
+                                                       int slices, int relu, float* __restrict__ amax_out, unsigned char* __restrict__ mask) {
+    const ColLane L = col_lane(rows, c4, tpr, cblocks, slices);
+    float am = 0.f;
+    if (L.live) {
+        const float4 mu = *reinterpret_cast<const float4*>(k.mean + L.c0);
+        const float4 is = *reinterpret_cast<const float4*>(k.invstd + L.c0);
+        const float4 ga = *reinterpret_cast<const float4*>(k.gamma + L.c0);
+        const float4 be = *reinterpret_cast<const float4*>(k.beta + L.c0);
+        am = bn_apply_rows<RES>(L, x, ldx, res, ldr, y, ldy, mu, is, ga, be, c4, relu, mask, false, 1.f);
+    }
+    if (amax_out) block_amax(am, amax_out);
+}
+
+constexpr int APPLY_MAX_C = 4096;
+template <bool RES>
+__global__ __launch_bounds__(256) void bn_apply_sums_kernel(const float* __restrict__ x, int ldx, const float* __restrict__ res, int ldr,
+                                                            float* __restrict__ y, int ldy, const double* __restrict__ sums, int rows, int c,
+                                                            float eps, float momentum, const float* __restrict__ gamma, const float* __restrict__ beta,
+                                                            float* __restrict__ mean_out, float* __restrict__ invstd_out, float* rmean, float* rvar,
+                                                            long long* nbt, int tpr, int cblocks, int slices, int relu, float* __restrict__ amax_out,
+                                                            unsigned char* __restrict__ mask, const float* __restrict__ colmax) {
+    __shared__ __attribute__((aligned(16))) float s_mean[APPLY_MAXCOL];
+    __shared__ __attribute__((aligned(16))) float s_is[APPLY_MAXCOL];
+    __shared__ float s_bound[4];
+    const int c4 = c >> 2;
+    const ColLane L = col_lane(rows, c4, tpr, cblocks, slices);
+    const int base = L.cb * tpr * 4, top = min(c, base + tpr * 4);
+    float bound = 0.f;
+    for (int ch = (colmax ? 0 : base) + threadIdx.x; ch < (colmax ? c : top); ch += blockDim.x) {
+        const double m = sums[ch] / rows;
+        double var = sums[c + ch] / rows - m * m;
+        if (var < 0) var = 0;
+        const float mf = (float)m, isf = (float)(1.0 / sqrt(var + (double)eps));
+        if (colmax) bound = fmaxf(bound, fabsf(gamma[ch]) * isf * (colmax[ch] + fabsf(mf)) + fabsf(beta[ch]));
+        if (ch >= base && ch < top) {
+            s_mean[ch - base] = mf; s_is[ch - base] = isf;
+            if (L.slice == 0) {
+                mean_out[ch] = mf; invstd_out[ch] = isf;
+                if (rmean) {
+                    const double unb = rows > 1 ? var * rows / (rows - 1) : var;
+                    rmean[ch] = (1.f - momentum) * rmean[ch] + momentum * (float)m;
+                    rvar[ch] = (1.f - momentum) * rvar[ch] + momentum * (float)unb;
+                }
+            }
+        }
+    }
+    if (blockIdx.x == 0 && threadIdx.x == 0 && nbt) *nbt += 1;
+    float sc = 1.f, sc_inv = 1.f;
+    if (colmax) {
+#pragma unroll
+        for (int o = 32; o > 0; o >>= 1) bound = fmaxf(bound, __shfl_xor(bound, o, 64));
+        if ((threadIdx.x & 63) == 0) s_bound[threadIdx.x >> 6] = bound;
+    }
+    __syncthreads();
+    if (colmax) {
+        bound = 1.0001f * fmaxf(fmaxf(s_bound[0], s_bound[1]), fmaxf(s_bound[2], s_bound[3]));
+        if (blockIdx.x == 0 && threadIdx.x == 0) *amax_out = bound;
+        pow2_scale(&bound, sc, sc_inv);
+    }
+    float am = 0.f;
+    if (L.live) {
+        const float4 mu = *reinterpret_cast<const float4*>(s_mean + (L.c0 - base));
+        const float4 is = *reinterpret_cast<const float4*>(s_is + (L.c0 - base));
+        const float4 ga = *reinterpret_cast<const float4*>(gamma + L.c0);
+        const float4 be = *reinterpret_cast<const float4*>(beta + L.c0);
+        am = bn_apply_rows<RES>(L, x, ldx, res, ldr, y, ldy, mu, is, ga, be, c4, relu, mask, colmax != nullptr, sc);
+    }
+    if (amax_out && !colmax) block_amax(am, amax_out);
+}
+
+struct BwdApply {
+    const float* dy; int lddy; const float* x; int ldx; const float* y; int ldy; Coef k;
+    const float* sum_dy; const float* sum_dyx;
+    float* dx; int lddx; float* dres; int lddres;
+    int rows, c, tpr, cblocks, slices, training; float inv_n;
+    float* amax_out; int packed; const unsigned char* mask; const float* dy2; int lddy2;
+    const double* fsums; const float* fmax; float* out_dbeta; float* out_dgamma;
+};
+template <bool HAS2, int RM, bool NEEDX>
+__global__ __launch_bounds__(256) void bn_bwd_apply_kernel(const BwdApply p) {
+    __shared__ float s_bound[4];
+    const int c = p.c, c4 = p.c >> 2;
+    const ColLane L = col_lane(p.rows, c4, p.tpr, p.cblocks, p.slices);
+    const int c0 = L.c0, cc = L.cc, rpp = L.rpp;
+    const int training = p.training, packed = p.packed;
+    const float inv_n = p.inv_n;
+    float am = 0.f, sc = 1.f, sc_inv = 1.f;
+    if (packed && p.fsums) {
+        float bound_local = 0.f;
+        for (int ch = threadIdx.x; ch < c; ch += blockDim.x) {
+            const float a = (float)p.fsums[ch], b = (float)p.fsums[c + ch];
+            const float kk = fabsf(p.k.gamma[ch] * p.k.invstd[ch]);
+            const float bb = 1.0001f * kk * (training ? p.fmax[ch] + inv_n * (fabsf(a) + p.fmax[c + ch] * fabsf(b)) : p.fmax[ch]);
+            if (bb < 3.0e38f) bound_local = fmaxf(bound_local, bb);
+        }
+#pragma unroll
+        for (int o = 32; o > 0; o >>= 1) bound_local = fmaxf(bound_local, __shfl_xor(bound_local, o, 64));
+        if ((threadIdx.x & 63) == 0) s_bound[threadIdx.x >> 6] = bound_local;
+        __syncthreads();
+        float bnd = fmaxf(fmaxf(s_bound[0], s_bound[1]), fmaxf(s_bound[2], s_bound[3]));
+        if (blockIdx.x == 0 && threadIdx.x == 0) *p.amax_out = bnd;
+        pow2_scale(&bnd, sc, sc_inv);
+    } else if (packed) pow2_scale(p.amax_out, sc, sc_inv);
+    if (L.live) {
+        const float4 is = *reinterpret_cast<const float4*>(p.k.invstd + c0);
+        const float4 ga = *reinterpret_cast<const float4*>(p.k.gamma + c0);
+        float4 mu = make_float4(0.f, 0.f, 0.f, 0.f), be = mu, s1 = mu, s2 = mu;
+        if (NEEDX) mu = *reinterpret_cast<const float4*>(p.k.mean + c0);
+        if (RM == 2) be = *reinterpret_cast<const float4*>(p.k.beta + c0);
+        if (p.fsums) {
+            s1 = make_float4((float)p.fsums[c0], (float)p.fsums[c0 + 1], (float)p.fsums[c0 + 2], (float)p.fsums[c0 + 3]);
+            s2 = make_float4((float)p.fsums[c + c0], (float)p.fsums[c + c0 + 1], (float)p.fsums[c + c0 + 2], (float)p.fsums[c + c0 + 3]);
+            if (L.slice == 0 && L.r == 0) {
+                if (p.out_dbeta) { p.out_dbeta[c0] = s1.x; p.out_dbeta[c0 + 1] = s1.y; p.out_dbeta[c0 + 2] = s1.z; p.out_dbeta[c0 + 3] = s1.w; }
+                if (p.out_dgamma) { p.out_dgamma[c0] = s2.x; p.out_dgamma[c0 + 1] = s2.y; p.out_dgamma[c0 + 2] = s2.z; p.out_dgamma[c0 + 3] = s2.w; }
+            }
+        } else if (training) {
+            s1 = *reinterpret_cast<const float4*>(p.sum_dy + c0);
+            s2 = *reinterpret_cast<const float4*>(p.sum_dyx + c0);
+        }
+        const float* __restrict__ dy = p.dy; const float* __restrict__ dy2 = p.dy2; const float* __restrict__ x = p.x;
+        const float* __restrict__ y = p.y; const unsigned char* __restrict__ mask = p.mask;
+        float* __restrict__ dx = p.dx; float* __restrict__ dres = p.dres;
+        const int lddy = p.lddy, lddy2 = p.lddy2, ldx = p.ldx, ldy = p.ldy, lddx = p.lddx, lddres = p.lddres;
+        auto emit = [&](long long row, float4 g, const float4 g2, const float4 xx, const float4 yy, unsigned m) __attribute__((always_inline)) {
+            if (HAS2) { g.x += g2.x; g.y += g2.y; g.z += g2.z; g.w += g2.w; }
+            if (RM == 1) {
+                g.x = (m & 1u) ? g.x : 0.f; g.y = (m & 2u) ? g.y : 0.f; g.z = (m & 4u) ? g.z : 0.f; g.w = (m & 8u) ? g.w : 0.f;
+            } else if (RM != 0) {
+                const float4 v = RM == 3 ? yy : make_float4(bn_val(xx.x, mu.x, is.x, ga.x, be.x), bn_val(xx.y, mu.y, is.y, ga.y, be.y),
+                                                            bn_val(xx.z, mu.z, is.z, ga.z, be.z), bn_val(xx.w, mu.w, is.w, ga.w, be.w));
+                g.x = v.x > 0.f ? g.x : 0.f; g.y = v.y > 0.f ? g.y : 0.f;
+                g.z = v.z > 0.f ? g.z : 0.f; g.w = v.w > 0.f ? g.w : 0.f;
+            }
+            if (dres) *reinterpret_cast<float4*>(dres + row * lddres + c0) = g;
+            float4 o;
+            if (training) {
+                o.x = ga.x * is.x * (g.x - inv_n * (s1.x + (xx.x - mu.x) * is.x * s2.x));
+                o.y = ga.y * is.y * (g.y - inv_n * (s1.y + (xx.y - mu.y) * is.y * s2.y));
+                o.z = ga.z * is.z * (g.z - inv_n * (s1.z + (xx.z - mu.z) * is.z * s2.z));
+                o.w = ga.w * is.w * (g.w - inv_n * (s1.w + (xx.w - mu.w) * is.w * s2.w));
+            } else {
+                o = make_float4(g.x * ga.x * is.x, g.y * ga.y * is.y, g.z * ga.z * is.z, g.w * ga.w * is.w);
+            }
+            if (packed) {
+                const SplitH sp = split4h(o, sc);
+                const float2 h = __builtin_bit_cast(float2, sp.h), l = __builtin_bit_cast(float2, sp.l);
+                o = make_float4(h.x, h.y, l.x, l.y);
+            } else {
+                am = fmaxf(fmaxf(am, fmaxf(fabsf(o.x), fabsf(o.y))), fmaxf(fabsf(o.z), fabsf(o.w)));
+            }
+            *reinterpret_cast<float4*>(dx + row * lddx + c0) = o;
+        };
+        int r = L.r;
+        for (; r + 3 * rpp < L.r1; r += 4 * rpp) {
+            float4 qg[4], qg2[4], qx[4], qy[4];
+            unsigned m[4] = {15u, 15u, 15u, 15u};
+#pragma unroll
+            for (int u = 0; u < 4; ++u) {
+                const long long row = r + u * rpp;
+                qg[u] = *reinterpret_cast<const float4*>(dy + row * lddy + c0);
+                if (HAS2) qg2[u] = *reinterpret_cast<const float4*>(dy2 + row * lddy2 + c0);
+                if (NEEDX) qx[u] = *reinterpret_cast<const float4*>(x + row * ldx + c0);
+                if (RM == 3) qy[u] = *reinterpret_cast<const float4*>(y + row * ldy + c0);
+                if (RM == 1) m[u] = mask[row * c4 + cc];
+            }
+            __builtin_amdgcn_sched_barrier(0);
+#pragma unroll
+            for (int u = 0; u < 4; ++u) emit(r + u * rpp, qg[u], HAS2 ? qg2[u] : qg[u], NEEDX ? qx[u] : mu, RM == 3 ? qy[u] : mu, m[u]);
+        }
+        for (; r < L.r1; r += rpp) {
+            const long long row = r;
+            const float4 qg = *reinterpret_cast<const float4*>(dy + row * lddy + c0);
+            const float4 qg2 = HAS2 ? *reinterpret_cast<const float4*>(dy2 + row * lddy2 + c0) : qg;
+            const float4 qx = NEEDX ? *reinterpret_cast<const float4*>(x + row * ldx + c0) : mu;
+            const float4 qy = RM == 3 ? *reinterpret_cast<const float4*>(y + row * ldy + c0) : mu;
+            const unsigned m = RM == 1 ? mask[row * c4 + cc] : 15u;
+            emit(row, qg, qg2, qx, qy, m);
+        }
+    }
+    if (p.amax_out && !packed) block_amax(am, p.amax_out);
+}
+
+int launch_bwd_apply(const BwdApply& p, int relu, hipStream_t s) {
+    const int rm = !relu ? 0 : (p.mask ? 1 : (p.y ? 3 : 2));
+    const bool needx = p.training || rm == 2;
+    const dim3 grid((unsigned)p.slices * (unsigned)p.cblocks);
+#define GLF_BNA(H2, RM_, NX) hipLaunchKernelGGL((bn_bwd_apply_kernel<H2, RM_, NX>), grid, dim3(256), 0, s, p)
+#define GLF_BNA_RM(H2, NX) do { if (rm == 0) GLF_BNA(H2, 0, NX); else if (rm == 1) GLF_BNA(H2, 1, NX); else GLF_BNA(H2, 3, NX); } while (0)
+    if (rm == 2) { if (p.dy2) GLF_BNA(true, 2, true); else GLF_BNA(false, 2, true); }
+    else if (p.dy2) { if (needx) GLF_BNA_RM(true, true); else GLF_BNA_RM(true, false); }
+    else { if (needx) GLF_BNA_RM(false, true); else GLF_BNA_RM(false, false); }
+#undef GLF_BNA_RM
+#undef GLF_BNA
+    return glf::check_launch("bn_bwd_apply");
 }
 
 constexpr int LN_NV = 8;
@@ -758,9 +846,11 @@
     GLF_REQUIRE(rows > 0, GLF_ERR_BAD_SHAPE, "bn_apply: rows must be > 0");
     REQ_C4(c); REQ_AL(x, "x"); REQ_AL(y, "y"); REQ_LD(ldx, "ldx"); REQ_LD(ldy, "ldy");
     if (residual) { REQ_AL(residual, "residual"); REQ_LD(ldr, "ldr"); }
-    const long long total4 = (long long)rows * (c / 4);
-    hipLaunchKernelGGL(bn_apply_kernel, dim3(stream_grid(total4, 256)), dim3(256), 0, glf::S(s), x, ldx, residual, ldr, y, ldy,
-                       Coef{mean, invstd, gamma, beta}, total4, c / 4, relu, amax_out, relu_mask);
+    const ColGrid g = col_grid(rows, c);
+#define GLF_BNF(RES_) hipLaunchKernelGGL((bn_apply_kernel<RES_>), col_dim(g), dim3(256), 0, glf::S(s), x, ldx, residual, ldr, y, ldy, \
+                                         Coef{mean, invstd, gamma, beta}, rows, c / 4, g.tpr, g.cblocks, g.slices, relu, amax_out, relu_mask)
+    if (residual) GLF_BNF(true); else GLF_BNF(false);
+#undef GLF_BNF
     return glf::check_launch("bn_apply");
 }
 
@@ -776,10 +866,12 @@
     GLF_REQUIRE(c <= APPLY_MAX_C, GLF_ERR_UNSUPPORTED, "bn_apply_from_sums: C must be <= %d (use glf_bn_stats_from_sums + glf_bn_apply)", APPLY_MAX_C);
     GLF_REQUIRE((running_mean == nullptr) == (running_var == nullptr), GLF_ERR_NULL, "bn_apply_from_sums: running_mean/var must both be set or both NULL");
     if (residual) { REQ_AL(residual, "residual"); REQ_LD(ldr, "ldr"); }
-    const long long total4 = (long long)rows * (c / 4);
-    hipLaunchKernelGGL(bn_apply_sums_kernel, dim3(stream_grid(total4, 256)), dim3(256), (size_t)2 * c * sizeof(float), glf::S(s), x, ldx, residual, ldr, y, ldy, sums, rows, c,
-                       eps, momentum, gamma, beta, mean, invstd, running_mean, running_var, reinterpret_cast<long long*>(num_batches_tracked),
-                       total4, c / 4, relu, amax_out, relu_mask, colmax);
+    const ColGrid g = col_grid(rows, c);
+#define GLF_BNF(RES_) hipLaunchKernelGGL((bn_apply_sums_kernel<RES_>), col_dim(g), dim3(256), 0, glf::S(s), x, ldx, residual, ldr, y, ldy, sums, rows, c, \
+                                         eps, momentum, gamma, beta, mean, invstd, running_mean, running_var,                                      \
+                                         reinterpret_cast<long long*>(num_batches_tracked), g.tpr, g.cblocks, g.slices, relu, amax_out, relu_mask, colmax)
+    if (residual) GLF_BNF(true); else GLF_BNF(false);
+#undef GLF_BNF
     return glf::check_launch("bn_apply_from_sums");
 }
 
@@ -799,7 +891,10 @@
     if (dres) { REQ_AL(dres, "dres"); REQ_LD(lddres, "lddres"); }
     if (dy2) { REQ_AL(dy2, "dy2"); REQ_LD(lddy2, "lddy2"); }
     const OpBnBwd op{dy, lddy, x, ldx, y, ldy, mean, invstd, gamma, beta, relu, relu_mask, c / 4, dy2, lddy2};
-    const long long total4f = (long long)rows * (c / 4);
+    const ColGrid ag = col_grid(rows, c);
+    BwdApply ap{dy, lddy, x, ldx, y, ldy, Coef{mean, invstd, gamma, beta}, nullptr, nullptr, dx, lddx, dres, lddres,
+                rows, c, ag.tpr, ag.cblocks, ag.slices, training, 1.0f / (float)rows,
+                amax_out, packed_dx, relu_mask, dy2, lddy2, nullptr, nullptr, nullptr, nullptr};
     const int phase = packed_dx >= 2 ? packed_dx : 0;
     GLF_REQUIRE(packed_dx >= 0 && packed_dx <= 3, GLF_ERR_BAD_SHAPE, "bn_bwd: packed_dx must be 0 .. 3");
     GLF_REQUIRE(!phase || (workspace && fused_sums), GLF_ERR_NULL, "bn_bwd: packed_dx = 2 / 3 needs the workspace and fused_sums (2 c floats kept from half 2 to half 3)");
@@ -812,15 +907,21 @@
         const dim3 rgrid(fs, (c4 + tpr - 1) / tpr);
         float* rmax = packed_dx ? fmax : (float*)nullptr;
         const int rm = !op.relu ? 0 : (op.mask ? 1 : (op.y ? 3 : 2));
-#define GLF_BNR(H2, RM_) hipLaunchKernelGGL((bnbwd_reduce_atomic_kernel<H2, RM_>), rgrid, dim3(RT), 0, glf::S(s), op, rows, c, fs, fused_sums, rmax)
-        if (op.dy2) { if (rm == 0) GLF_BNR(true, 0); else if (rm == 1) GLF_BNR(true, 1); else if (rm == 2) GLF_BNR(true, 2); else GLF_BNR(true, 3); }
-        else { if (rm == 0) GLF_BNR(false, 0); else if (rm == 1) GLF_BNR(false, 1); else if (rm == 2) GLF_BNR(false, 2); else GLF_BNR(false, 3); }
+        const bool wres = dy2 && dres;
+        GLF_REQUIRE(!wres || (dres != dy && dres != dy2 && dres != x), GLF_ERR_BAD_SHAPE, "bn_bwd: dres must not alias dy, dy2 or x");
+#define GLF_BNR(H2, RM_, WR) hipLaunchKernelGGL((bnbwd_reduce_atomic_kernel<H2, RM_, WR>), rgrid, dim3(RT), 0, glf::S(s), op, rows, c, fs, fused_sums, rmax, \
+                                                (WR) ? dres : (float*)nullptr, lddres)
+        if (wres) { if (rm == 0) GLF_BNR(true, 0, true); else if (rm == 1) GLF_BNR(true, 1, true); else if (rm == 2) GLF_BNR(true, 2, true); else GLF_BNR(true, 3, true); }
+        else if (op.dy2) { if (rm == 0) GLF_BNR(true, 0, false); else if (rm == 1) GLF_BNR(true, 1, false); else if (rm == 2) GLF_BNR(true, 2, false); else GLF_BNR(true, 3, false); }
+        else { if (rm == 0) GLF_BNR(false, 0, false); else if (rm == 1) GLF_BNR(false, 1, false); else if (rm == 2) GLF_BNR(false, 2, false); else GLF_BNR(false, 3, false); }
 #undef GLF_BNR
         if (int rc = glf::check_launch("bn_bwd_reduce(fused)")) return rc;
-        hipLaunchKernelGGL(bn_bwd_apply_kernel, dim3(stream_grid(total4f, 256)), dim3(256), (size_t)2 * c * sizeof(float), glf::S(s), dy, lddy, x, ldx, y, ldy,
-                           Coef{mean, invstd, gamma, beta}, (const float*)nullptr, (const float*)nullptr, dx, lddx, dres, lddres, total4f, c / 4, relu, training,
-                           1.0f / (float)rows, amax_out, packed_dx, relu_mask, dy2, lddy2, fused_sums, fmax, dbeta, dgamma, c);
-        return glf::check_launch("bn_bwd_apply(fused)");
+        ap.fsums = fused_sums; ap.fmax = fmax; ap.out_dbeta = dbeta; ap.out_dgamma = dgamma;
+        if (wres) {
+            ap.dy = dres; ap.lddy = lddres; ap.dy2 = nullptr; ap.mask = nullptr; ap.y = nullptr; ap.dres = nullptr;
+            return launch_bwd_apply(ap, 0, glf::S(s));
+        }
+        return launch_bwd_apply(ap, relu, glf::S(s));
     }
     GLF_REQUIRE(workspace, GLF_ERR_NULL, "bn_bwd: the three-launch form needs the workspace");
     const int slices = n_slices_c(rows, c);
@@ -842,12 +943,8 @@
     }
     if (int rc = glf::check_launch("bn_bwd_finalize")) return rc;
     if (phase == 2) return GLF_OK;
-    const long long total4 = (long long)rows * (c / 4);
-    hipLaunchKernelGGL(bn_bwd_apply_kernel, dim3(stream_grid(total4, 256)), dim3(256), 0, glf::S(s), dy, lddy, x, ldx, y, ldy,
-                       Coef{mean, invstd, gamma, beta}, s_dy, s_dyx, dx, lddx, dres, lddres, total4, c / 4, relu, training,
-                       1.0f / (float)rows, amax_out, packed_dx, relu_mask, dy2, lddy2, (const double*)nullptr, (const float*)nullptr, (float*)nullptr,
-                       (float*)nullptr, c);
-    return glf::check_launch("bn_bwd_apply");
+    ap.sum_dy = s_dy; ap.sum_dyx = s_dyx;
+    return launch_bwd_apply(ap, relu, glf::S(s));
 }
 
 extern "C" int glf_colsum(const float* dy, int lddy, float* db, int rows, int c, double* workspace, glf_stream_t s) {
diff --git a/profiles/ubench/bn_stream_probe.py b/profiles/ubench/bn_stream_probe.py
--- /dev/null
+++ b/profiles/ubench/bn_stream_probe.py
@@ -0,0 +1,149 @@
+#!/usr/bin/env python3
+import argparse
+import ctypes as C
+import os
+import statistics
+import sys
+
+import numpy as np
+import torch
+
+sys.path.insert(0, os.path.join(os.path.dirname(os.path.abspath(__file__)), "..", ".."))
+from glfusion_amd import ops
+from glfusion_amd._lib import lib, check
+
+DEV = torch.device("cuda", 0)
+SHAPES = [(193600, 64), (193600, 256), (50176, 256), (50176, 512), (50176, 1024), (50176, 2048)]
+EPS, MOM = 1e-5, 0.1
+
+
+def p(t):
+    return None if t is None else t.data_ptr()
+
+
+def rnd(rows, c, seed, scale=1.0, shift=0.0):
+    g = torch.Generator(device=DEV).manual_seed(seed)
+    return torch.rand(rows, c, generator=g, device=DEV) * (2.0 * scale) - scale + shift
+
+
+def timed(fn, reset=None, n=10, warm=3):
+    ts = []
+    for i in range(warm + n):
+        if reset is not None:
+            reset()
+        a, b = torch.cuda.Event(enable_timing=True), torch.cuda.Event(enable_timing=True)
+        a.record()
+        fn()
+        b.record()
+        b.synchronize()
+        if i >= warm:
+            ts.append(a.elapsed_time(b))
+    return statistics.median(ts), max(ts) - min(ts)
+
+
+def main():
+    ap = argparse.ArgumentParser()
+    ap.add_argument("--save")
+    ap.add_argument("--compare")
+    ap.add_argument("--pair-only", action="store_true")
+    args = ap.parse_args()
+    ops.set_precision("f16x3")
+    print(f"library: {os.environ.get('GLF_LIB_PATH', 'default')}")
+    keep_dir = args.save or args.compare
+    if args.save:
+        os.makedirs(args.save, exist_ok=True)
+    mismatches = []
+
+    def record(tag, **tensors):
+        if not keep_dir:
+            return
+        for name, t in tensors.items():
+            path = os.path.join(keep_dir, f"{tag}_{name}.npy")
+            a = t.detach().cpu().contiguous().view(torch.uint8).numpy()
+            if args.save:
+                np.save(path, a)
+            else:
+                same = np.array_equal(np.load(path), a)
+                print(f"    {tag} {name}: {'bit-identical' if same else 'DIFFERS'}")
+                if not same:
+                    mismatches.append(f"{tag} {name}")
+
+    shapes = [(50176, 256), (50176, 1024)] if args.pair_only else SHAPES
+    for rows, c in shapes:
+        n = rows * c
+        x = rnd(rows, c, 1, 2.0, 0.3)
+        res = rnd(rows, c, 2)
+        dy, dy2 = rnd(rows, c, 3, 3.0), rnd(rows, c, 4, 0.7)
+        gamma, beta = rnd(1, c, 5, 0.5, 1.0).view(c), rnd(1, c, 6).view(c)
+        sums = torch.stack([x.double().sum(0), (x.double() ** 2).sum(0)]).contiguous()
+        colmax = x.abs().amax(0).contiguous()
+        y, pk, dx, dres = (torch.empty(rows, c, device=DEV) for _ in range(4))
+        mask = torch.empty(rows * (c // 4), dtype=torch.uint8, device=DEV)
+        mean, invstd = torch.empty(c, device=DEV), torch.empty(c, device=DEV)
+        rm, rv, nbt = torch.zeros(c, device=DEV), torch.ones(c, device=DEV), torch.zeros((), dtype=torch.int64, device=DEV)
+        am = torch.zeros(1, device=DEV)
+        dg, db = torch.empty(c, device=DEV), torch.empty(c, device=DEV)
+        fs = torch.zeros(3 * c, dtype=torch.float64, device=DEV)
+        keep = torch.empty(2 * c, device=DEV)
+        ws = torch.empty(int(lib.glf_bn_workspace(rows, c)), dtype=torch.float64, device=DEV)
+        print(f"rows x C = {rows} x {c}  ({n * 4 / 1e6:.0f} MB per fp32 tensor)")
+
+        def report(name, bytes_per_el, t, spread, alt=None):
+            extra = f"   ({alt * n / t / 1e6:7.0f} GB/s at {alt} B / element)" if alt else ""
+            print(f"  {name:44s} {t * 1e3:8.1f} us  spread {spread * 1e3:5.1f}  {bytes_per_el * n / t / 1e6:7.0f} GB/s at {bytes_per_el} B / element{extra}")
+
+        def fwd_inner():
+            check(lib.glf_bn_apply_from_sums(p(x), c, None, c, p(pk), c, p(sums), rows, c, EPS, MOM, p(gamma), p(beta), p(mean), p(invstd),
+                                             p(rm), p(rv), p(nbt), 1, p(am), None, p(colmax), None), "fwd inner")
+
+        def fwd_last():
+            check(lib.glf_bn_apply_from_sums(p(x), c, p(res), c, p(y), c, p(sums), rows, c, EPS, MOM, p(gamma), p(beta), p(mean), p(invstd),
+                                             p(rm), p(rv), p(nbt), 1, p(am), p(mask), None, None), "fwd last")
+
+        def bwd_inner():
+            check(lib.glf_bn_bwd(p(dy), c, p(x), c, None, c, p(mean), p(invstd), p(gamma), p(beta), p(dx), c, None, c, p(dg), p(db),
+                                 rows, c, 1, 1, None, p(am), 1, None, None, 0, p(fs), None), "bwd inner")
+
+        def bwd_last():
+            check(lib.glf_bn_bwd(p(dy), c, p(x), c, None, c, p(mean), p(invstd), p(gamma), p(beta), p(dx), c, p(dres), c, p(dg), p(db),
+                                 rows, c, 1, 1, None, p(am), 1, p(mask), p(dy2), c, p(fs), None), "bwd last")
+
+        def bwd_phase(phase):
+            check(lib.glf_bn_bwd(p(dy), c, p(x), c, None, c, p(mean), p(invstd), p(gamma), p(beta), p(dx), c, None, c,
+                                 p(dg) if phase == 2 else None, p(db) if phase == 2 else None,
+                                 rows, c, 1, 1, p(ws), p(am), phase, None, None, 0, p(keep), None), "bwd phase")
+
+        def zero():
+            fs.zero_(); am.zero_()
+
+        arr = (C.c_void_p * 2)(dy.data_ptr(), dy2.data_ptr())
+
+        def add_n():
+            check(lib.glf_add_n(arr, 2, p(dres), n, None), "add_n")
+
+        if not args.pair_only:
+            am.zero_(); fwd_inner(); torch.cuda.synchronize()
+            record(f"{rows}x{c}_fwd_inner", image=pk, bound=am, mean=mean, invstd=invstd, rmean=rm, rvar=rv)
+            report("fwd inner (packed out)", 8, *timed(fwd_inner, am.zero_))
+            am.zero_(); fwd_last(); torch.cuda.synchronize()
+            record(f"{rows}x{c}_fwd_last", y=y, mask=mask, amax=am, mean=mean, invstd=invstd)
+            report("fwd last (residual, ReLU, sign bytes)", 12.25, *timed(fwd_last, am.zero_))
+            zero(); bwd_inner(); torch.cuda.synchronize()
+            record(f"{rows}x{c}_bwd_inner", image=dx)
+            report("bwd inner pair (packed dx)", 20, *timed(bwd_inner, zero))
+        zero(); fwd_last(); zero(); bwd_last(); torch.cuda.synchronize()
+        record(f"{rows}x{c}_bwd_last", dres=dres)
+        report("bwd last pair (dy + dy2, bytes, dres, packed)", 32.5, *timed(bwd_last, zero), alt=28.25)
+        if not args.pair_only:
+            am.zero_(); bwd_phase(2); bwd_phase(3); torch.cuda.synchronize()
+            record(f"{rows}x{c}_bwd_apply", image=dx, bound=am)
+            report("bwd apply alone (packed dx)", 12, *timed(lambda: bwd_phase(3)))
+            report("add_n, two addends", 12, *timed(add_n))
+        del x, res, dy, dy2, y, pk, dx, dres, ws
+        torch.cuda.empty_cache()
+    if args.compare:
+        print("bit-identity against the saved outputs: " + ("ALL bit-identical" if not mismatches else f"{len(mismatches)} differ: {mismatches}"))
+
+
+if __name__ == "__main__":
+    main()
```

After: 17.56 clips/s, median of 6. 1.02x the previous value.
